# qingpingmo/OCN

Measured on AMD Instinct MI355X. Metric: candidate-edges/sec (CN predictor fwd), ogbl-collab shape, higher is better.
Workload: dtype f32

## Files before the change

### include/ocn_hip.h

```cpp
#ifndef OCN_HIP_H
#define OCN_HIP_H

#include <stdint.h>

#ifdef __cplusplus
extern "C" {
#endif

#define OCN_ABI_VERSION 9
#define OCN_EINVAL (-1)
#define OCN_ECAP   (-2)

#define OCN_ST_CAP  1
#define OCN_ST_SCAN 2
#define OCN_SCAN_POISON (-1)

#define OCN_F_CN1 1u
#define OCN_F_CN2 2u

int ocn_abi_version(void);

int64_t ocn_scan_workspace_bytes(int64_t n);

int ocn_zero_regions(void* const* ptrs, const int64_t* bytes, int32_t n, void* stream);

int ocn_edge_offsets(const int64_t* rowptrA, const int64_t* src, int64_t B,
                     int64_t* off, void* workspace, void* stream);

int ocn_check_edges(const int64_t* src, const int64_t* dst, int64_t B, int64_t n_src, int64_t n_dst,
                    int32_t* bad, void* stream);

int64_t ocn_order_workspace_bytes(int64_t n_nodes);
int ocn_order_by_node(const int64_t* node, int64_t B, int64_t n_nodes, int64_t* order, void* workspace,
                      void* stream);

int ocn_batch_prep(const int64_t* rowptrA, const int64_t* src, int64_t B, int64_t* off , void* scan_workspace,
                   int64_t n_nodes, void* order_workspace , void* const* zero_ptrs, const int64_t* zero_bytes,
                   int32_t n_zero, void* stream);
int ocn_order_by_node_finish(const int64_t* node, int64_t B, int64_t n_nodes, int64_t* order, void* workspace,
                             void* stream);
int ocn_order_by_node_finish_rec(const int64_t* node , const int64_t* dst, const int64_t* rowptrA,
                                 const int64_t* off, int64_t B, int64_t n_nodes, int64_t* order, uint64_t* rec ,
                                 void* workspace, void* stream);

int ocn_chunk_offsets(const int64_t* rowptrA, const int64_t* nds , const int64_t* src,
                      const int64_t* order, int64_t B, int64_t* out, void* workspace, void* stream);

#define OCN_CLASS_RANGES 7
int ocn_class_order(const int32_t* cnt1, const int32_t* cnt2 , const int64_t* order_in ,
                    int64_t B, int64_t* order_out, int64_t* inv_out, int64_t* ranges, int64_t* prefix,
                    void* workspace, void* stream);

int ocn_scan_i32(const int32_t* in, int64_t n, int64_t* out, void* workspace, void* stream);

int ocn_cn_flags(const int64_t* rowptrA, const int32_t* colA,
                 const int64_t* rowptrT1, const int32_t* colT1,
                 const int64_t* rowptrT2, const int32_t* colT2,
                 const uint32_t* bitmapT1 , int64_t bm1_stride_words,
                 const uint32_t* bitmapT2 , int64_t bm_stride_words,
                 const int64_t* src, const int64_t* dst, const int64_t* order, int64_t B,
                 int64_t n_cols, const int64_t* off, uint8_t* flags, int64_t flags_cap,
                 uint64_t* hist , int32_t* cnt1, int32_t* cnt2,
                 int32_t* status, uint64_t* rec , int32_t* gcost , void* stream);
int ocn_cn_flags_rec(const int64_t* rowptrA, const int32_t* colA,
                     const int64_t* rowptrT1, const int32_t* colT1,
                     const int64_t* rowptrT2, const int32_t* colT2,
                     const uint32_t* bitmapT1 , int64_t bm1_stride_words,
                     const uint32_t* bitmapT2 , int64_t bm_stride_words,
                     const int64_t* src, const int64_t* dst, const int64_t* order, int64_t B,
                     int64_t n_cols, const int64_t* off, uint8_t* flags, int64_t flags_cap,
                     uint64_t* hist , int32_t* cnt1, int32_t* cnt2,
                     int32_t* status, uint64_t* rec , int32_t* gcost , void* stream);

int32_t ocn_walk_chunk(void);
int ocn_cn_walk_flags(const int64_t* rowptrA, const int32_t* colA, const int64_t* nds ,
                      const int64_t* src, const int64_t* dst, const int64_t* order, int64_t B,
                      const int64_t* chunk_off, const int64_t* rev_off , const int64_t* off,
                      int64_t max_row_len ,
                      uint8_t* flags, int32_t* wc, int64_t flags_cap,
                      uint64_t* hist , int32_t* cnt1, int32_t* cnt2,
                      int32_t* status, void* stream);

int ocn_neighbor_degree_sum(const int64_t* rowptr, const int32_t* col, int64_t n_rows, int64_t* out,
                            void* stream);
int ocn_walk_rev_offsets(const int64_t* rowptrA, const int64_t* nds, const int64_t* src, const int64_t* dst,
                         const int64_t* order, int64_t B, int64_t* out , void* workspace,
                         void* stream);

int32_t ocn_walk_prep_max_batch(void);
int ocn_walk_prep(const int64_t* rowptrA, const int64_t* nds , const int64_t* src, const int64_t* dst,
                  int64_t B, int32_t min_share, int64_t* order, int64_t* off, int64_t* chunk_off,
                  int64_t* rev_off , int32_t* g_head , int64_t* g_item_off ,
                  int32_t* g_active , int32_t* meta, int32_t* cnt1,
                  int32_t* cnt2, int32_t* status, int32_t* scal, void* stream);
int ocn_cn_walk_group(const int64_t* rowptrA, const int32_t* colA, const int64_t* src, const int64_t* dst,
                      const int64_t* order, int64_t B, const int32_t* g_head, const int64_t* g_item_off,
                      const int32_t* g_active, int32_t* meta, const int64_t* off, uint8_t* flags, int32_t* wc,
                      int64_t flags_cap, uint64_t* hist, int32_t* cnt1, int32_t* cnt2, void* stream);

int ocn_cn_weights_cn5(uint64_t* hist, int64_t N, const float* innerprod, int32_t* scalars,
                       int32_t valued, const float* s2_exact , void* stream);
int ocn_cn_weights_cn7(uint64_t* hist, int64_t N, float sum_fill, const float* diag1 ,
                       const float* diag2 , void* stream);

int ocn_cn5_column_stats(const uint64_t* hist, int64_t N, int32_t* scalars, void* stream);

int64_t ocn_cn_colsum_workspace_bytes(int64_t N, int64_t flags_cap);
int ocn_cn_colsum_exact(const int64_t* rowptrA, const int32_t* colA, const int64_t* src, int64_t B,
                        const int64_t* off, const uint8_t* flagsA, const uint8_t* flagsB ,
                        const int32_t* wc , int64_t flags_cap, const uint64_t* hist ,
                        int64_t N, const float* innerprod, int32_t* scalars, const float* s2_init ,
                        float* s2 , float* s3 , void* workspace, void* stream);

int ocn_cn_gather(const int64_t* rowptrA, const int32_t* colA,
                  const int64_t* src, const int64_t* dst, const int64_t* order, int64_t B,
                  const int64_t* off, const uint8_t* flags, const int32_t* wc,
                  const float* weights , const float* h, int32_t H, int64_t max_row_len,
                  float* xcn1, float* xcn2, float* xij, const int64_t* out_row,
                  const int32_t* cnt1, const int32_t* cnt2, const uint64_t* rec ,
                  const int32_t* perm , const float* rowsum ,
                  void* stream);
int ocn_cn8_pool(const int64_t* rowptrA, const int32_t* colA,
                 const int64_t* rowptrT1 , const int32_t* colT1 ,
                 const int64_t* rowptrT2 , const int32_t* colT2 ,
                 const uint32_t* bitmapT1 , int64_t bm1_stride_words,
// ... 113 lines not shown
int ocn_combine3(const float* coef, const float* x1, const float* x2, const float* x3, int64_t n,
                 float* out, void* stream);

int ocn_fill_rows(float* dst, int64_t ld, int32_t n_cols, const float* vec, const int64_t* row_range,
                  int64_t max_rows, void* stream);

typedef struct OcnLinearGroup {
  const float* X; int64_t ldX;
  int64_t M;
  const void* Wp;
  const float* bias;
  const float* gamma; const float* beta; float eps;
  int32_t relu;
  const float* scale;
  const float* addend; int64_t ldAdd;
  const float* dotw; const float* dotb;
  float* Y; int64_t ldY;
  const int64_t* row_range;
  const int64_t* y_row_map;
  int32_t add_bcast;
} OcnLinearGroup;

int64_t ocn_linear_panel_bytes(int32_t N, int32_t K);
int ocn_linear_split_weight(const float* W, int32_t N, int32_t K, void* Wp, void* stream);
int ocn_linear_bf16x6(const float* X, int64_t M, int32_t K, const void* Wp, int32_t N,
                      const float* bias, const float* gamma, const float* beta, float eps,
                      int32_t relu, const float* dotw, const float* dotb, float* Y, void* stream);
int ocn_linear_grouped(const OcnLinearGroup* groups, int32_t n_groups, int32_t K, int32_t N, void* stream);

typedef struct OcnHeadsArgs {
  const float* x[3];
  int64_t ldx, B;
  int32_t H;
  const void* p_first[3];
  const void* p_mid[2];
  const void* p_out[3];
  const float* vec;
  const int64_t* ranges;
  const int64_t* y_row_map;
  float* y;
  float* dump;
  const float* cpark;
  float* scratch;
  float eps;
  int32_t ln, b_on_union;
} OcnHeadsArgs;
int32_t ocn_heads_nvec(void);
int32_t ocn_heads_nscal(void);
int64_t ocn_heads_scratch_bytes(int32_t H);
int64_t ocn_heads_const_bytes(int32_t H);
int64_t ocn_heads_panel_bytes(int32_t N, int32_t K);
int ocn_heads_split_weight(const float* W, int32_t N, int32_t K, float scale, void* Wp, void* stream);
int ocn_heads_fused(const OcnHeadsArgs* args, void* stream);
int64_t ocn_heads_small_batch(int64_t max_rows);

int64_t ocn_coo_to_csr_workspace_bytes(int64_t nnz, int64_t n_rows, int32_t symmetrize, int32_t dedupe);
int ocn_coo_to_csr(const int64_t* row, const int64_t* col, int64_t nnz, int64_t n_rows, int64_t n_cols,
                   int32_t symmetrize, int32_t dedupe, int64_t* rowptr, int32_t* col_out, void* workspace,
                   int64_t* result, void* stream);

int64_t ocn_wgrad_workspace_bytes(int64_t B, int32_t N, int32_t K);
int ocn_wgrad(const float* dY, int64_t ldY, const float* X, int64_t ldX, int64_t B, int32_t N, int32_t K,
              float* dW, float* db, void* workspace, void* stream);

int64_t ocn_ln_drop_relu_workspace_bytes(int32_t H);
int ocn_ln_drop_relu_forward(const float* x, const float* gamma , const float* beta , float eps, float p,
                             uint64_t seed, int32_t relu, int64_t rows, int32_t H, float* y, float* stats ,
                             void* stream);
int ocn_ln_drop_relu_backward(const float* g, const float* x, const float* y, const float* stats, const float* gamma ,
                              float p, uint64_t seed, int32_t relu, int64_t rows, int32_t H, float* dx,
                              float* dgamma, float* dbeta, void* workspace, void* stream);
int ocn_dropout_keep_mask(uint64_t seed, float p, int64_t n, uint8_t* out, void* stream);

int64_t ocn_mix3_workspace_bytes(void);
int ocn_mix3_backward(const float* coef, const float* g, const float* x1, const float* x2, const float* x3, int64_t n,
                      float* d1, float* d2, float* d3, float* dcoef, void* workspace, void* stream);

#ifdef __cplusplus
}
#endif
#endif
```

### ocn_amd/_lib.py

```python
from __future__ import annotations

import ctypes
import glob
import os
import subprocess
from ctypes import c_float, c_int32, c_int64, c_void_p

_HERE = os.path.dirname(os.path.abspath(__file__))
_ROOT = os.path.dirname(_HERE)
LIB_PATH = os.environ.get("OCN_LIB_PATH", os.path.join(_HERE, "libocn_hip.so"))
CSRC = os.path.join(_HERE, "csrc")
INCLUDE = os.path.join(_ROOT, "include")

_P = c_void_p
ABI_VERSION = 9
SIGNATURES = {
    "ocn_abi_version": (c_int32, []),
    "ocn_scan_workspace_bytes": (c_int64, [c_int64]),
    "ocn_zero_regions": (c_int32, [_P, _P, c_int32, _P]),
    "ocn_check_edges": (c_int32, [_P, _P, c_int64, c_int64, c_int64, _P, _P]),
    "ocn_edge_offsets": (c_int32, [_P, _P, c_int64, _P, _P, _P]),
    "ocn_class_order": (c_int32, [_P, _P, _P, c_int64, _P, _P, _P, _P, _P, _P]),
    "ocn_scan_i32": (c_int32, [_P, c_int64, _P, _P, _P]),
    "ocn_order_workspace_bytes": (c_int64, [c_int64]),
    "ocn_order_by_node": (c_int32, [_P, c_int64, c_int64, _P, _P, _P]),
    "ocn_order_by_node_finish": (c_int32, [_P, c_int64, c_int64, _P, _P, _P]),
    "ocn_order_by_node_finish_rec": (c_int32, [_P, _P, _P, _P, c_int64, c_int64, _P, _P, _P, _P]),
    "ocn_batch_prep": (c_int32, [_P, _P, c_int64, _P, _P, c_int64, _P, _P, _P, c_int32, _P]),
    "ocn_cn_flags": (c_int32, [_P, _P, _P, _P, _P, _P, _P, c_int64, _P, c_int64, _P, _P, _P, c_int64, c_int64, _P, _P, c_int64, _P,
                               _P, _P, _P, _P, _P, _P]),
    "ocn_cn_flags_rec": (c_int32, [_P, _P, _P, _P, _P, _P, _P, c_int64, _P, c_int64, _P, _P, _P, c_int64, c_int64, _P, _P, c_int64, _P,
                                   _P, _P, _P, _P, _P, _P]),
    "ocn_chunk_offsets": (c_int32, [_P, _P, _P, _P, c_int64, _P, _P, _P]),
    "ocn_walk_chunk": (c_int32, []),
    "ocn_cn_walk_flags": (c_int32, [_P, _P, _P, _P, _P, _P, c_int64, _P, _P, _P, c_int64, _P, _P, c_int64, _P, _P, _P,
                                    _P, _P]),
    "ocn_neighbor_degree_sum": (c_int32, [_P, _P, c_int64, _P, _P]),
    "ocn_walk_prep_max_batch": (c_int32, []),
    "ocn_cn_flags_small_graph_cols": (c_int32, []),
    "ocn_walk_prep": (c_int32, [_P, _P, _P, _P, c_int64, c_int32, _P, _P, _P, _P, _P, _P, _P, _P, _P, _P, _P, _P, _P]),
    "ocn_cn_walk_group": (c_int32, [_P, _P, _P, _P, _P, c_int64, _P, _P, _P, _P, _P, _P, _P, c_int64, _P, _P, _P, _P]),
    "ocn_walk_rev_offsets": (c_int32, [_P, _P, _P, _P, _P, c_int64, _P, _P, _P]),
    "ocn_cn_weights_cn5": (c_int32, [_P, c_int64, _P, _P, c_int32, _P, _P]),
    "ocn_cn5_column_stats": (c_int32, [_P, c_int64, _P, _P]),
    "ocn_cn_colsum_workspace_bytes": (c_int64, [c_int64, c_int64]),
    "ocn_cn_colsum_exact": (c_int32, [_P, _P, _P, c_int64, _P, _P, _P, _P, c_int64, _P, c_int64, _P, _P, _P, _P, _P, _P, _P]),
    "ocn_cn_weights_cn7": (c_int32, [_P, c_int64, c_float, _P, _P, _P]),
    "ocn_cn_gather": (c_int32, [_P, _P, _P, _P, _P, c_int64, _P, _P, _P, _P, _P, c_int32, c_int64, _P, _P, _P, _P, _P,
                                _P, _P, _P, _P, _P]),
    "ocn_cn8_pool": (c_int32, [_P, _P, _P, _P, _P, _P, _P, c_int64, _P, c_int64, _P, _P, _P, c_int64, c_int64, _P, c_int32, _P, _P,
                               _P, _P, _P, _P]),
    "ocn_cn_node_sums": (c_int32, [_P, _P, _P, _P, _P, _P, _P, c_int64, _P, c_int64, _P, _P, _P, c_int64, c_int64, _P, _P, _P, _P, _P,
                                   _P, _P]),
    "ocn_row_diff_stage_cols": (c_int32, []),
    "ocn_row_diff_count": (c_int32, [_P, _P, _P, _P, _P, c_int64, c_int32, _P, _P]),
    "ocn_row_diff_fill": (c_int32, [_P, _P, _P, _P, _P, c_int64, c_int32, _P, _P, _P]),
    "ocn_two_hop_window_cols": (c_int64, []),
    "ocn_two_hop_diff_count": (c_int32, [_P, _P, _P, _P, c_int64, _P, c_int64, c_int32, c_int64, _P, _P]),
    "ocn_two_hop_diff_fill": (c_int32, [_P, _P, _P, _P, c_int64, _P, c_int64, c_int32, c_int64, _P, _P, _P]),
    "ocn_segment_topk_max_k": (c_int32, []),
    "ocn_segment_topk": (c_int32, [_P, _P, c_int64, c_int32, _P, _P, _P]),
    "ocn_philox4x32": (c_int32, [_P, ctypes.c_uint32, ctypes.c_uint32, c_int64, _P, _P]),
    "ocn_complement_count": (c_int32, [_P, _P, c_int64, _P, _P]),
    "ocn_sample_stage_cols": (c_int32, []),
    "ocn_sample_complement_rows": (c_int32, [_P, _P, c_int64, _P, c_int64, c_int64, c_int64, ctypes.c_uint64, _P, _P]),
    "ocn_sample_complement_pairs": (c_int32, [_P, _P, c_int64, _P, c_int64, c_int64, ctypes.c_uint64, _P, _P]),
    "ocn_gather_schedule": (c_int32, [_P, c_int64, c_int64, _P, _P]),
    "ocn_coo_to_csr_workspace_bytes": (c_int64, [c_int64, c_int64, c_int32, c_int32]),
    "ocn_coo_to_csr": (c_int32, [_P, _P, c_int64, c_int64, c_int64, c_int32, c_int32, _P, _P, _P, _P, _P]),
    "ocn_wgrad_workspace_bytes": (c_int64, [c_int64, c_int32, c_int32]),
    "ocn_wgrad": (c_int32, [_P, c_int64, _P, c_int64, c_int64, c_int32, c_int32, _P, _P, _P, _P]),
    "ocn_cn_weights_cn6": (c_int32, [_P, _P, c_int64, _P, _P, _P, _P, _P, _P]),
    "ocn_cn_gather3": (c_int32, [_P, _P, _P, _P, _P, c_int64, _P, _P, _P, _P, _P, _P, _P, c_int32, _P, _P, _P, _P, _P]),
    "ocn_cn_gather3_backward": (c_int32, [_P, _P, _P, _P, _P, c_int64, _P, _P, _P, _P, _P, _P, _P, c_int32, _P, _P, _P, _P, _P, _P]),
    "ocn_cn_gather_backward": (c_int32, [_P, _P, _P, _P, _P, c_int64, _P, _P, _P, _P, _P, c_int32, _P, _P, _P, _P, _P]),
    "ocn_cn_gather_backward_det_workspace_bytes": (c_int64, [c_int64, c_int64, c_int64]),
    "ocn_cn_gather_backward_det": (c_int32, [_P, _P, _P, _P, c_int64, _P, _P, _P, c_int64, _P, _P, c_int64, c_int32, _P, _P, _P, _P,
                                             _P, _P]),
    "ocn_cn_gather_backward_det_keys_offset": (c_int64, [c_int64]),
    "ocn_cn_gather_backward_det_lists": (c_int32, [_P, _P, _P, _P, c_int64, _P, _P, c_int64, c_int64, _P, _P]),
    "ocn_ln_drop_relu_workspace_bytes": (c_int64, [c_int32]),
    "ocn_ln_drop_relu_forward": (c_int32, [_P, _P, _P, c_float, c_float, ctypes.c_uint64, c_int32, c_int64, c_int32, _P, _P, _P]),
    "ocn_ln_drop_relu_backward": (c_int32, [_P, _P, _P, _P, _P, c_float, ctypes.c_uint64, c_int32, c_int64, c_int32, _P, _P, _P, _P, _P]),
    "ocn_dropout_keep_mask": (c_int32, [ctypes.c_uint64, c_float, c_int64, _P, _P]),
    "ocn_mix3_workspace_bytes": (c_int64, []),
    "ocn_mix3_backward": (c_int32, [_P, _P, _P, _P, _P, c_int64, _P, _P, _P, _P, _P, _P]),
    "ocn_spmm_csr": (c_int32, [_P, _P, _P, c_int64, _P, c_int32, _P, _P, c_int32, c_int32, c_int32, _P, _P]),
    "ocn_spmm_csr_max_arg": (c_int32, [_P, _P, _P, c_int64, _P, c_int32, _P, _P, _P]),
    "ocn_spmm_max_backward": (c_int32, [_P, _P, _P, c_int64, _P, _P, c_int32, _P, _P]),
    "ocn_deg_rsqrt": (c_int32, [_P, _P, c_int64, c_float, _P, _P]),
    "ocn_spgemm_max_cols": (c_int64, []),
    "ocn_spgemm_pattern_count": (c_int32, [_P, _P, c_int64, _P, _P, c_int64, _P, _P, c_int64, _P]),
    "ocn_spgemm_pattern_fill": (c_int32, [_P, _P, c_int64, _P, _P, c_int64, _P, _P, _P]),
    "ocn_spgemm_bit_rows": (c_int32, [_P, _P, c_int64, _P, _P, c_int64, _P, c_int64, _P, _P, c_int64, _P]),
    "ocn_dense_from_csr": (c_int32, [_P, _P, c_int64, c_int64, _P, _P, _P]),
    "ocn_dense_block_mm_bits": (c_int32, [_P, _P, c_int64, c_int64, c_int32, c_int32, c_int32, c_int32, c_int32, _P, c_int64, _P]),
    "ocn_bitrows_from_csr": (c_int32, [_P, _P, c_int64, _P, c_int64, _P]),
    "ocn_bitrows_count": (c_int32, [_P, c_int64, c_int64, c_int64, _P, _P]),
    "ocn_bitrows_fill": (c_int32, [_P, c_int64, c_int64, c_int64, _P, _P, _P]),
    "ocn_rows_ln_relu": (c_int32, [_P, _P, _P, c_float, c_int32, c_int64, c_int32, _P, _P]),
    "ocn_fill_rows": (c_int32, [_P, c_int64, c_int32, _P, _P, c_int64, _P]),
    "ocn_combine3": (c_int32, [_P, _P, _P, _P, c_int64, _P, _P]),
    "ocn_linear_panel_bytes": (c_int64, [c_int32, c_int32]),
    "ocn_linear_split_weight": (c_int32, [_P, c_int32, c_int32, _P, _P]),
    "ocn_linear_bf16x6": (c_int32, [_P, c_int64, c_int32, _P, c_int32, _P, _P, _P, c_float, c_int32, _P, _P,
                                    _P, _P]),
    "ocn_linear_grouped": (c_int32, [_P, c_int32, c_int32, c_int32, _P]),
    "ocn_heads_nvec": (c_int32, []),
    "ocn_heads_nscal": (c_int32, []),
    "ocn_heads_scratch_bytes": (c_int64, [c_int32]),
    "ocn_heads_const_bytes": (c_int64, [c_int32]),
    "ocn_heads_panel_bytes": (c_int64, [c_int32, c_int32]),
    "ocn_heads_split_weight": (c_int32, [_P, c_int32, c_int32, c_float, _P, _P]),
    "ocn_heads_fused": (c_int32, [_P, _P]),
    "ocn_heads_small_batch": (c_int64, [c_int64]),
}


class OcnHipError(RuntimeError):
    pass


class OcnLinearGroup(ctypes.Structure):
    _fields_ = [("X", c_void_p), ("ldX", c_int64), ("M", c_int64), ("Wp", c_void_p), ("bias", c_void_p),
                ("gamma", c_void_p), ("beta", c_void_p), ("eps", c_float), ("relu", c_int32),
                ("scale", c_void_p), ("addend", c_void_p), ("ldAdd", c_int64), ("dotw", c_void_p),
                ("dotb", c_void_p), ("Y", c_void_p), ("ldY", c_int64), ("row_range", c_void_p),
                ("y_row_map", c_void_p), ("add_bcast", c_int32)]


class OcnHeadsArgs(ctypes.Structure):
    _fields_ = [("x", c_void_p * 3), ("ldx", c_int64), ("B", c_int64), ("H", c_int32),
                ("p_first", c_void_p * 3), ("p_mid", c_void_p * 2), ("p_out", c_void_p * 3),
                ("vec", c_void_p), ("ranges", c_void_p), ("y_row_map", c_void_p), ("y", c_void_p),
                ("dump", c_void_p), ("cpark", c_void_p), ("scratch", c_void_p), ("eps", c_float), ("ln", c_int32), ("b_on_union", c_int32)]


def sources():
    return sorted(glob.glob(os.path.join(CSRC, "*.hip")))


def build_flags():
    return ["-O3", "--offload-arch=gfx950", "-fPIC", "-std=c++17",
            "-ffp-contract=off",
            "-frecord-command-line",
            f"-I{INCLUDE}", f"-I{CSRC}"]


def build(force: bool = False, verbose: bool = False, jobs: int = None) -> str:
    import hashlib
    from concurrent.futures import ThreadPoolExecutor
    out = LIB_PATH
    hdrs = sorted(glob.glob(os.path.join(CSRC, "*.h"))) + [os.path.join(INCLUDE, "ocn_hip.h")]
    deps = sources() + hdrs + [os.path.abspath(__file__)]
    if not force and os.path.exists(out) and \
            os.path.getmtime(out) >= max(os.path.getmtime(d) for d in deps):
        return out
    hipcc = os.environ.get("HIPCC", "/opt/rocm/bin/hipcc")
    flags = build_flags()
    tag = hashlib.sha1(" ".join(flags).encode()).hexdigest()[:10]
    bdir = os.path.join(CSRC, "_build", tag)
    os.makedirs(bdir, exist_ok=True)
    hdr_time = max(os.path.getmtime(h) for h in hdrs)
    todo, objs = [], []
    for src in sources():
        obj = os.path.join(bdir, os.path.basename(src)[:-4] + ".o")
        objs.append(obj)
# ... 52 lines not shown
```

### ocn_amd/csrc/cn_stage.hip

```cpp
#include "common.h"


template <typename P>
__device__ __forceinline__ bool sorted_has(P a, i64 n, int32_t key) {
  i64 lo = 0, hi = n;
  bool found = false;
  while (lo < hi) {
    const i64 mid = (lo + hi) >> 1;
    const int32_t v = a[mid];
    found |= (v == key);
    if (v < key) lo = mid + 1; else hi = mid;
  }
  return found;
}

__device__ __forceinline__ bool sampled_has(const int32_t* samp, const int32_t* __restrict__ row, i64 n,
                                            int32_t key) {
  int lo = 0, hi = OCN_WAVE;
  while (lo < hi) {
    const int mid = (lo + hi) >> 1;
    if (samp[mid] <= key) lo = mid + 1; else hi = mid;
  }
  if (lo == 0) return false;
  const int s = lo - 1;
  const i64 p0 = ((i64)s * n) >> 6, p1 = ((i64)(s + 1) * n) >> 6;
  return sorted_has(row + p0, p1 - p0, key);
}

#define T1_CAP 1024
#define REC_FULL2_BIT 61
#define SCHED_COST(t, c) ((t) > (c) ? (t) : (c))
constexpr int SCHED_SHIFT = 5;
constexpr int POOL_LPE = 64;
#define SCHED_GROUP OCN_WPB

#define LH_MAX_COLS 8192

__device__ __forceinline__ void wave_lds_sync() {
  __builtin_amdgcn_fence(__ATOMIC_ACQ_REL, "wavefront");
  __builtin_amdgcn_wave_barrier();
}
__device__ __forceinline__ i64 wave_uniform(i64 v) {
  const unsigned lo = __builtin_amdgcn_readfirstlane((unsigned)(u64)v), hi = __builtin_amdgcn_readfirstlane((unsigned)((u64)v >> 32));
  return (i64)(((u64)hi << 32) | lo);
}
__device__ __forceinline__ bool lanes_have(int32_t t, int32_t key) {
  int pos = 0;
#pragma unroll
  for (int step = OCN_WAVE / 2; step > 0; step >>= 1)
    if (__shfl(t, pos + step - 1, OCN_WAVE) < key) pos += step;
  return __shfl(t, pos, OCN_WAVE) == key;
}

template <bool HAS_T2, bool LH, bool RECIN>
__global__ __launch_bounds__(OCN_BLOCK) void cn_flags_kernel(
    const i64* __restrict__ rowptrA, const int32_t* __restrict__ colA,
    const i64* __restrict__ rowptrT1, const int32_t* __restrict__ colT1,
    const i64* __restrict__ rowptrT2, const int32_t* __restrict__ colT2,
    const unsigned* __restrict__ bmT1, i64 bm1_stride, const unsigned* __restrict__ bmT2, i64 bm_stride,
    const i64* __restrict__ src, const i64* __restrict__ dst, const i64* __restrict__ order, i64 B,
    i64 n_cols, const i64* __restrict__ off, uint8_t* __restrict__ flags, i64 cap,
    u64* __restrict__ hist, int32_t* __restrict__ cnt1, int32_t* __restrict__ cnt2,
    int32_t* __restrict__ status, u64* rec, int32_t* __restrict__ gcost) {
  constexpr int GPB = OCN_WPB;
  __shared__ int s_cost[2][GPB];
  __shared__ int32_t s_t1[GPB][T1_CAP];
  __shared__ int32_t s_t2[GPB][OCN_WAVE];
  extern __shared__ __attribute__((aligned(16))) u64 s_hist[];
  const int gl = threadIdx.x % OCN_WAVE, g = __builtin_amdgcn_readfirstlane(threadIdx.x / OCN_WAVE);
  if (blockIdx.x == 0 && threadIdx.x == 0) status_raise(status, off[B], cap);
  const bool void_batch = off[B] < 0;
  if (LH) {
    for (i64 c = threadIdx.x; c < n_cols; c += OCN_BLOCK) s_hist[c] = 0ull;
    __syncthreads();
  }
  int par = 0;
  for (i64 e0 = (i64)blockIdx.x * GPB; e0 < B; e0 += (i64)gridDim.x * GPB, par ^= 1) {
    const i64 slot = e0 + g;
    const bool act = slot < B;
    i64 e = 0, i = 0, j = 0, a0 = 0, da = 0, b0 = 0, db = 0, c0 = 0, dc = 0, base = 0;
    const unsigned* bm_row = nullptr;
    const unsigned* bm1_row = nullptr;
    if (act) {
      if (RECIN) {
        const ulonglong2* rp = reinterpret_cast<const ulonglong2*>(rec + 4 * slot);
        const ulonglong2 ra = rp[0], rb = rp[1];
        e = wave_uniform((i64)ra.x);
        i = wave_uniform((i64)(ra.y & 0xffffffffull)); j = wave_uniform((i64)(ra.y >> 32));
        a0 = wave_uniform((i64)(rb.x & ((1ull << REC_LEN_SHIFT) - 1))); da = wave_uniform((i64)(rb.x >> REC_LEN_SHIFT));
        base = wave_uniform((i64)rb.y);
      } else {
        e = order ? order[slot] : slot;
        i = src[e]; j = dst[e];
        a0 = rowptrA[i]; da = rowptrA[i + 1] - a0;
        base = off[e];
      }
      if (bmT1) bm1_row = bmT1 + j * bm1_stride;
      else { b0 = rowptrT1[j]; db = rowptrT1[j + 1] - b0; }
      if (HAS_T2) {
        if (bmT2) bm_row = bmT2 + j * bm_stride;
        if (rowptrT2 && (LH || !bmT2)) { c0 = rowptrT2[j]; dc = rowptrT2[j + 1] - c0; }
      }
      if (void_batch) { da = 0; db = 0; dc = 0; base = 0; }
    }
    const bool t1_reg = db <= OCN_WAVE, t1_lds = db <= T1_CAP;
    int32_t t1 = 0x7fffffff;
    if (t1_reg) { if (gl < db) t1 = colT1[b0 + gl]; }
    else if (t1_lds)
      for (i64 q = gl; q < db; q += OCN_WAVE) s_t1[g][q] = colT1[b0 + q];
    const bool t2_full = HAS_T2 && rowptrT2 && dc == n_cols;
    if (HAS_T2 && !t2_full && !bmT2) {
      if (dc > OCN_WAVE) s_t2[g][gl] = colT2[c0 + (((i64)gl * dc) >> 6)];
      else if (gl < dc) s_t2[g][gl] = colT2[c0 + gl];
    }
    wave_lds_sync();
    const bool fits = base + da <= cap;
    int c1 = 0, c2 = 0;
    for (i64 p0 = 0; p0 < da; p0 += OCN_WAVE) {
      const i64 p = p0 + gl;
      const bool in = p < da;
      const int32_t k = in ? colA[a0 + p] : 0;
      unsigned w2 = 0;
      if (HAS_T2 && bmT2 && !t2_full && in) w2 = bm_row[k >> 5];
      bool f1;
      if (bmT1) f1 = in && ((bm1_row[k >> 5] >> (k & 31)) & 1u);
      else if (t1_reg) f1 = lanes_have(t1, k) && in;
      else f1 = in && (t1_lds ? sorted_has(&s_t1[g][0], db, k) : sorted_has(colT1 + b0, db, k));
      bool f2 = false;
      if (HAS_T2 && in) {
        if (t2_full) f2 = true;
        else if (bmT2) f2 = (w2 >> (k & 31)) & 1u;
        else f2 = dc > OCN_WAVE ? sampled_has(&s_t2[g][0], colT2 + c0, dc, k) : sorted_has(&s_t2[g][0], dc, k);
      }
      if (fits && in) flags[base + p] = (uint8_t)((f1 ? OCN_F_CN1 : 0u) | (f2 ? OCN_F_CN2 : 0u));
      if (f1 | f2) {
        const u64 inc = (u64)f1 | ((u64)f2 << HF_BITS) | (1ull << (2 * HF_BITS));
        if (LH) atomicAdd(s_hist + k, inc); else atomicAdd(hist + 2 * (i64)k, inc);
      }
      c1 += f1;
      c2 += f2;
    }
    wave_lds_sync();
#pragma unroll
    for (int o = OCN_WAVE / 2; o > 0; o >>= 1) {
      c1 += __shfl_xor(c1, o, OCN_WAVE);
      c2 += __shfl_xor(c2, o, OCN_WAVE);
    }
    if (act && gl == 0) {
      cnt1[e] = c1;
      if (cnt2) cnt2[e] = c2;
      if (rec) {
        u64* r = rec + 4 * slot;
        if (!RECIN) {
          r[0] = (u64)e;
          r[1] = (u64)i | ((u64)j << 32);
        }
        if (!RECIN || void_batch) r[2] = (u64)a0 | ((u64)da << REC_LEN_SHIFT);
        r[3] = (u64)base | ((u64)(da > 0 && (i64)c2 == da) << REC_FULL2_BIT) | ((u64)(c1 > 0) << 62) | ((u64)(c2 > 0) << 63);
      }
    }
    if (gcost) {
      if (gl == 0) s_cost[par][g] = act ? c1 + c2 : 0;
      __syncthreads();
      if (threadIdx.x == 0) {
        int t = 0;
#pragma unroll
        for (int q = 0; q < GPB; ++q) t = SCHED_COST(t, s_cost[par][q]);
// ... 425 lines not shown
      const bool need = (wa[t] != 0.f) | (wb[t] != 0.f);
      unsigned long long m = __ballot(need);
      if (LPE < 64) m = (m >> gbase) & ((1ull << (LPE & 63)) - 1ull);
      while (m) {
        int bsel[UNR];
#pragma unroll
        for (int u = 0; u < UNR; ++u) {
          bsel[u] = m ? (__ffsll((long long)m) - 1) : -1;
          m &= m - 1;
        }
        int32_t kk[UNR];
        float wwa[UNR], wwb[UNR];
        float4 x[UNR][NV];
#pragma unroll
        for (int u = 0; u < UNR; ++u) {
          const int sl = gbase + (bsel[u] < 0 ? 0 : bsel[u]);
          kk[u] = __shfl(k[t], sl, OCN_WAVE);
          wwa[u] = __shfl(wa[t], sl, OCN_WAVE);
          wwb[u] = __shfl(wb[t], sl, OCN_WAVE);
          if (bsel[u] >= 0) {
            const float4* row = h4 + (i64)kk[u] * rowq + gl;
#pragma unroll
            for (int v = 0; v < NV; ++v) x[u][v] = row[v * LPE];
          }
        }
#pragma unroll
        for (int u = 0; u < UNR; ++u) {
          if (bsel[u] >= 0) {
            const f32x2 w = {wwa[u], wwb[u]};
#pragma unroll
            for (int v = 0; v < NV; ++v) {
              axpy_pair(acc[v][0], w, x[u][v].x);
              axpy_pair(acc[v][1], w, x[u][v].y);
              axpy_pair(acc[v][2], w, x[u][v].z);
              axpy_pair(acc[v][3], w, x[u][v].w);
            }
          }
        }
      }
    }
  }
#pragma unroll
  for (int v = 0; v < NV; ++v) {
    acc1[v] = make_float4(acc[v][0].x, acc[v][1].x, acc[v][2].x, acc[v][3].x);
    acc2[v] = make_float4(acc[v][0].y, acc[v][1].y, acc[v][2].y, acc[v][3].y);
  }
}

template <int LPE, int NV>
__device__ __forceinline__ void pool_store(i64 e, i64 i, i64 j, int gl, const float4* __restrict__ h4, i64 rowq,
                                           const float4 (&acc1)[NV], const float4 (&acc2)[NV],
                                           float* __restrict__ xcn1, float* __restrict__ xcn2,
                                           float* __restrict__ xij, bool st1 = true, bool st2 = true) {
  const float4* hi = h4 + i * rowq + gl;
  const float4* hj = h4 + j * rowq + gl;
  float4* o1 = reinterpret_cast<float4*>(xcn1) + e * rowq + gl;
  float4* o2 = reinterpret_cast<float4*>(xcn2) + e * rowq + gl;
  float4* o3 = reinterpret_cast<float4*>(xij) + e * rowq + gl;
#pragma unroll
  for (int v = 0; v < NV; ++v) {
    const float4 a = hi[v * LPE], b = hj[v * LPE];
    if (st1) o1[v * LPE] = acc1[v];
    if (st2) o2[v * LPE] = acc2[v];
    o3[v * LPE] = make_float4(__fmul_rn(a.x, b.x), __fmul_rn(a.y, b.y), __fmul_rn(a.z, b.z),
                              __fmul_rn(a.w, b.w));
  }
}

#define LONG_ROW 1024

template <int LPE, int NV>
__global__ __launch_bounds__(OCN_BLOCK) void cn_gather_kernel(
    const i64* __restrict__ rowptrA, const int32_t* __restrict__ colA,
    const i64* __restrict__ src, const i64* __restrict__ dst, const i64* __restrict__ order, i64 B,
    const i64* __restrict__ off, const uint8_t* __restrict__ flags, const int32_t* __restrict__ wc,
    const float4* __restrict__ weights, const float* __restrict__ h, int H,
    float* __restrict__ xcn1, float* __restrict__ xcn2, float* __restrict__ xij,
    const i64* __restrict__ out_row,
    const int32_t* __restrict__ cnt1, const int32_t* __restrict__ cnt2,
    const u64* __restrict__ rec,
    const int32_t* __restrict__ perm,
    const float* __restrict__ rowsum) {
  constexpr int GPW = OCN_WAVE / LPE;
  const int lane = threadIdx.x & 63;
  const int gl = lane % LPE;
  const int gbase = lane - gl;
  i64 bid = blockIdx.x;
  if ((gridDim.x & 7) == 0) {
    bid = (bid & 7) * (gridDim.x >> 3) + (bid >> 3);
    if (perm) bid = perm[bid];
  }
  const i64 slot = (bid * OCN_WPB + (threadIdx.x >> 6)) * GPW + lane / LPE;
  if (slot >= B) return;
  i64 e, i, j, a0, da, base;
  bool has1, has2, full2;
  if (rec) {
    const ulonglong2* rp = reinterpret_cast<const ulonglong2*>(rec + 4 * slot);
    const ulonglong2 ra = rp[0], rb = rp[1];
    e = (i64)ra.x; i = (i64)(ra.y & 0xffffffffull); j = (i64)(ra.y >> 32);
    a0 = (i64)(rb.x & ((1ull << REC_LEN_SHIFT) - 1)); da = (i64)(rb.x >> REC_LEN_SHIFT);
    base = (i64)(rb.y & ((1ull << REC_FULL2_BIT) - 1)); has1 = (rb.y >> 62) & 1ull; has2 = rb.y >> 63;
    full2 = rowsum && ((rb.y >> REC_FULL2_BIT) & 1ull);
  } else {
    e = order ? order[slot] : slot;
    i = src[e]; j = dst[e];
    a0 = rowptrA[i]; da = rowptrA[i + 1] - a0;
    base = off[e];
    has1 = !cnt1 || cnt1[e] > 0; has2 = !cnt2 || cnt2[e] > 0;
    full2 = rowsum && cnt2 && da > 0 && (i64)cnt2[e] == da;
  }
  if (da > LONG_ROW && !full2) return;
  const float4* h4 = reinterpret_cast<const float4*>(h);
  const i64 rowq = H >> 2;
  float4 acc1[NV], acc2[NV];
#pragma unroll
  for (int v = 0; v < NV; ++v) acc1[v] = acc2[v] = make_float4(0.f, 0.f, 0.f, 0.f);
  if (has1 | (has2 & !full2)) pool_range<LPE, NV>(0, da, a0, base, gl, gbase, colA, flags, wc, weights, h4, rowq, acc1, acc2, full2);
  if (full2) {
    const float4* rs = reinterpret_cast<const float4*>(rowsum) + i * rowq + gl;
#pragma unroll
    for (int v = 0; v < NV; ++v) acc2[v] = rs[v * LPE];
  }
  pool_store<LPE, NV>(out_row ? out_row[e] : e, i, j, gl, h4, rowq, acc1, acc2, xcn1, xcn2, xij,
                      !out_row || has1, !out_row || has1 || has2);
}

template <int FPL, int HF>
__device__ __forceinline__ void chain_rows(const float2* __restrict__ w, const float* __restrict__ xs, int nr,
                                           float (&acc1)[FPL], float (&acc2)[FPL]) {
  constexpr int BLK = FPL >= 4 ? 2 : 8 / FPL;
  f32x2 acc[FPL];
#pragma unroll
  for (int q = 0; q < FPL; ++q) acc[q] = f32x2{acc1[q], acc2[q]};
  auto load = [&](int r, float2 (&w8)[BLK], float (&x8)[BLK][FPL]) {
#pragma unroll
    for (int u = 0; u < BLK; ++u) {
      w8[u] = w[r + u];
#pragma unroll
      for (int q = 0; q < FPL; ++q) x8[u][q] = xs[(r + u) * HF + q];
    }
  };
  auto add = [&](const float2 (&w8)[BLK], const float (&x8)[BLK][FPL]) {
#pragma unroll
    for (int u = 0; u < BLK; ++u)
#pragma unroll
      for (int q = 0; q < FPL; ++q) axpy_pair_lds(acc[q], f32x2{w8[u].x, w8[u].y}, x8[u][q]);
  };
  const int nb = nr / BLK;
  if (nb > 0) {
    float2 wa[BLK], wb[BLK];
    float xa[BLK][FPL], xb[BLK][FPL];
    load(0, wa, xa);
    int b = 0;
    for (; b + 2 <= nb; b += 2) {
      load((b + 1) * BLK, wb, xb);
      add(wa, xa);
      if (b + 2 < nb) load((b + 2) * BLK, wa, xa);
      add(wb, xb);
    }
    if (b < nb) add(wa, xa);
  }
  for (int r = nb * BLK; r < nr; ++r) {
    const float2 wr = w[r];
#pragma unroll
// ... 179 lines not shown
    if (f) entry_weights(f, weights[k], (float)cv, wa, wb);
    const bool need = (wa != 0.f) | (wb != 0.f);
    const unsigned long long m = __ballot(need);
    if (lane == 0) s_wcnt[wv] = __popcll(m);
    __syncthreads();
    int before = 0, n = 0;
#pragma unroll
    for (int q = 0; q < WAVES; ++q) {
      const int c = s_wcnt[q];
      if (q < wv) before += c;
      n += c;
    }
    if (need) {
      const int rank = before + __popcll(m & ((1ull << lane) - 1ull));
      s_k[rank] = k;
      s_w[rank] = make_float2(wa, wb);
    }
    __syncthreads();
    const int nsr = (n + SLAB - 1) / SLAB;
    f32x4 xa[RPG][NV], xb[RPG][NV];
    if (wv > 0) {
      long_request<LPE, NV, RPG, FG, SLAB>(xa, s_k, 0, n, fg, gl, h4, rowq);
      long_request<LPE, NV, RPG, FG, SLAB>(xb, s_k, 1, n, fg, gl, h4, rowq);
    }
    for (int t = -1; t < nsr; t += 2) {
      if (wv > 0) {
        long_store<LPE, NV, RPG, FG, SLAB>(xa, s_x + (size_t)((t + 1) & 1) * SLAB * ROWQ, n - (t + 1) * SLAB, fg, gl);
        long_request<LPE, NV, RPG, FG, SLAB>(xa, s_k, t + 3, n, fg, gl, h4, rowq);
      } else if (t >= 0 && lane < AL) {
        const int r0 = t * SLAB;
        chain_rows<FPL, HF>(s_w + r0, reinterpret_cast<const float*>(s_x + (size_t)(t & 1) * SLAB * ROWQ) + lane * FPL,
                            n - r0 < SLAB ? n - r0 : SLAB, acc1, acc2);
      }
      __syncthreads();
      if (t + 1 < nsr) {
        if (wv > 0) {
          long_store<LPE, NV, RPG, FG, SLAB>(xb, s_x + (size_t)((t + 2) & 1) * SLAB * ROWQ, n - (t + 2) * SLAB, fg, gl);
          long_request<LPE, NV, RPG, FG, SLAB>(xb, s_k, t + 4, n, fg, gl, h4, rowq);
        } else if (lane < AL) {
          const int r0 = (t + 1) * SLAB;
          chain_rows<FPL, HF>(s_w + r0, reinterpret_cast<const float*>(s_x + (size_t)((t + 1) & 1) * SLAB * ROWQ) + lane * FPL,
                              n - r0 < SLAB ? n - r0 : SLAB, acc1, acc2);
        }
        __syncthreads();
      }
    }
  }
  if (wv == 0 && lane < AL) {
    const i64 o = (out_row ? out_row[e] : e) * H + lane * FPL;
#pragma unroll
    for (int q = 0; q < FPL; ++q) {
      xcn1[o + q] = acc1[q];
      xcn2[o + q] = acc2[q];
      xij[o + q] = __fmul_rn(h[i * H + lane * FPL + q], h[j * H + lane * FPL + q]);
    }
  }
}

template <int LPE, int NV>
__global__ __launch_bounds__(OCN_BLOCK) void cn_gather3_kernel(
    const i64* __restrict__ rowptrA, const int32_t* __restrict__ colA,
    const i64* __restrict__ src, const i64* __restrict__ dst, const i64* __restrict__ order, i64 B,
    const i64* __restrict__ off, const uint8_t* __restrict__ flagsA, const uint8_t* __restrict__ flagsB,
    const float4* __restrict__ wA, const float4* __restrict__ wB, const float* __restrict__ nip_p,
    const float* __restrict__ h, int H, float* __restrict__ xcn1, float* __restrict__ xcn2,
    float* __restrict__ xcn3, float* __restrict__ xij) {
  constexpr int GPW = OCN_WAVE / LPE;
  constexpr int UNR = 4;
  const int lane = threadIdx.x & 63;
  const int gl = lane % LPE;
  const int gbase = lane - gl;
  const i64 slot = ((i64)blockIdx.x * OCN_WPB + (threadIdx.x >> 6)) * GPW + lane / LPE;
  if (slot >= B) return;
  const i64 e = order ? order[slot] : slot;
  const i64 i = src[e], j = dst[e];
  const i64 a0 = rowptrA[i], da = rowptrA[i + 1] - a0;
  const i64 base = off[e];
  const float nip = nip_p[0];
  const float4* h4 = reinterpret_cast<const float4*>(h);
  const i64 rowq = H >> 2;
  float4 acc1[NV], acc2[NV], acc3[NV];
#pragma unroll
  for (int v = 0; v < NV; ++v) acc1[v] = acc2[v] = acc3[v] = make_float4(0.f, 0.f, 0.f, 0.f);
  for (i64 p0 = 0; p0 < da; p0 += LPE) {
    const i64 p = p0 + gl;
    int32_t k = 0;
    unsigned fa = 0, fb = 0;
    if (p < da) { k = colA[a0 + p]; fa = flagsA[base + p]; fb = flagsB[base + p] & OCN_F_CN1; }
    float w1 = 0.f, w2 = 0.f, w3 = 0.f;
    if (fa | fb) {
      const float4 a = wA[k];
      const float inv3 = wB[k].x;
      const float tt = (fa & OCN_F_CN1) ? a.y : 0.f;
      w1 = (fa & OCN_F_CN1) ? a.x : 0.f;
      w2 = __fmul_rn(__fsub_rn((fa & OCN_F_CN2) ? 1.0f : 0.f, tt), a.z);
      w3 = __fmul_rn(__fsub_rn(__fsub_rn(fb ? 1.0f : 0.f, tt), __fmul_rn(nip, w2)), inv3);
    }
    const bool need = (w1 != 0.f) | (w2 != 0.f) | (w3 != 0.f);
    unsigned long long m = __ballot(need);
    if (LPE < 64) m = (m >> gbase) & ((1ull << (LPE & 63)) - 1ull);
    while (m) {
      int bsel[UNR];
#pragma unroll
      for (int u = 0; u < UNR; ++u) {
        bsel[u] = m ? (__ffsll((long long)m) - 1) : -1;
        m &= m - 1;
      }
// ... 224 lines not shown
      hipLaunchKernelGGL((cn_gather_wave_kernel<LPE, NV>), dim3((unsigned)((B + WW - 1) / WW)),
                         dim3(WW * OCN_WAVE), 0, st, (const i64*)rowptrA, colA, (const i64*)src, (const i64*)dst,
                         (const i64*)order, (i64)B, (const i64*)off, flags, wc, (const float4*)weights, h, (int)H,
                         xcn1, xcn2, xij, (const i64*)out_row, cnt2, rowsum);
      packed = false;
    }
  }
#define PACKED_ARGS (const i64*)rowptrA, colA, (const i64*)src, (const i64*)dst, (const i64*)order, (i64)B, \
                    (const i64*)off, flags, wc, (const float4*)weights, h, (int)H, xcn1, xcn2, xij,           \
                    (const i64*)out_row, cnt1, cnt2, (const u64*)rec
  if (packed)
    hipLaunchKernelGGL((cn_gather_kernel<LPE, NV>), dim3((unsigned)((B + epb - 1) / epb)), dim3(OCN_BLOCK), 0, st,
                       PACKED_ARGS, sched ? perm : (const int32_t*)nullptr, rowsum);
#undef PACKED_ARGS
#define LONG_ARGS (const i64*)rowptrA, colA, (const i64*)src, (const i64*)dst, (i64)B, (const i64*)off, flags, wc, \
                  (const float4*)weights, h, (int)H, xcn1, xcn2, xij, (const i64*)out_row, cnt2, rowsum
  if (max_row_len > LONG_ROW) {
    bool small = false;
    if constexpr (NV == 1) {
      if (B <= 4096) {
        static bool raised_dev[64] = {};
        int devid = 0;
        if (hipGetDevice(&devid) == hipSuccess && devid >= 0 && devid < 64 && !raised_dev[devid]) {
          if (hipFuncSetAttribute((const void*)cn_gather_long_kernel<LPE, NV, LONG_SMALL_THREADS>, hipFuncAttributeMaxDynamicSharedMemorySize,
                                  2 * LONG_SLAB_BYTES(LONG_SMALL_THREADS)) == hipSuccess) raised_dev[devid] = true;
        }
        hipLaunchKernelGGL((cn_gather_long_kernel<LPE, NV, LONG_SMALL_THREADS>), dim3((unsigned)B), dim3(LONG_SMALL_THREADS), 2 * LONG_SLAB_BYTES(LONG_SMALL_THREADS), st, LONG_ARGS);
        small = true;
      }
    }
    if (!small) {
      bool by_wave = false;
      if constexpr (LPE <= 16) {
        hipLaunchKernelGGL((cn_gather_wave_kernel<LPE, NV, true>), dim3((unsigned)B), dim3(OCN_WAVE), 0, st, (const i64*)rowptrA, colA, (const i64*)src, (const i64*)dst,
                           (const i64*)order, (i64)B, (const i64*)off, flags, wc, (const float4*)weights, h, (int)H,
                           xcn1, xcn2, xij, (const i64*)out_row, cnt2, rowsum);
        by_wave = true;
      }
      if (!by_wave) hipLaunchKernelGGL((cn_gather_long_kernel<LPE, NV, 256>), dim3((unsigned)B), dim3(256), 2 * LONG_SLAB_BYTES(256), st, LONG_ARGS);
    }
  }
#undef LONG_ARGS
}

extern "C" {

int32_t ocn_cn_flags_small_graph_cols(void) { return LH_MAX_COLS; }

static int cn_flags_launch(const int64_t* rowptrA, const int32_t* colA, const int64_t* rowptrT1,
                           const int32_t* colT1, const int64_t* rowptrT2, const int32_t* colT2,
                           const uint32_t* bitmapT1, int64_t bm1_stride_words, const uint32_t* bitmapT2, int64_t bm_stride_words,
                           const int64_t* src, const int64_t* dst, const int64_t* order, int64_t B,
                           int64_t n_cols, const int64_t* off, uint8_t* flags, int64_t flags_cap, uint64_t* hist,
                           int32_t* cnt1, int32_t* cnt2, int32_t* status, uint64_t* rec, int32_t* gcost, bool rec_in, void* stream) {
  if (B < 0 || flags_cap < 0 || B > (int64_t)HF_MASK) return OCN_EINVAL;
  if (B == 0) return 0;
  if (!rowptrA || (!rowptrT1 && !bitmapT1) || !src || !dst || !off || !hist || !cnt1 || !status) return OCN_EINVAL;
  if (rec_in && (!rec || !order)) return OCN_EINVAL;
  if ((bitmapT1 && bm1_stride_words * 32 < n_cols) || (bitmapT2 && bm_stride_words * 32 < n_cols)) return OCN_EINVAL;
  constexpr int GPB = OCN_WPB;
  hipStream_t st = (hipStream_t)stream;
  const bool lh = n_cols > 0 && n_cols <= LH_MAX_COLS;
  const size_t lds = lh ? (size_t)n_cols * sizeof(u64) : 0;
  const int grid = lh ? grid_for((B + GPB - 1) / GPB, 256 * 3) : grid_for((B + GPB - 1) / GPB);
  if (lh) {
    static bool raised_dev[64] = {};
    int devid = 0;
    if (hipGetDevice(&devid) != hipSuccess || devid < 0 || devid >= 64) return OCN_EINVAL;
    bool& raised = raised_dev[devid];
    if (!raised) {
      const void* fns[4] = {(const void*)cn_flags_kernel<true, true, false>, (const void*)cn_flags_kernel<false, true, false>,
                            (const void*)cn_flags_kernel<true, true, true>, (const void*)cn_flags_kernel<false, true, true>};
      for (const void* fn : fns) {
        hipError_t e1 = hipFuncSetAttribute(fn, hipFuncAttributeMaxDynamicSharedMemorySize, LH_MAX_COLS * (int)sizeof(u64));
        if (e1 != hipSuccess) return (int)e1;
      }
      raised = true;
    }
  }
#define CN_FLAGS_ARGS(T2P, T2C)                                                                      \
  (const i64*)rowptrA, colA, (const i64*)rowptrT1, colT1, (const i64*)(T2P), (T2C),                   \
      (const unsigned*)bitmapT1, (i64)bm1_stride_words, (const unsigned*)bitmapT2, (i64)bm_stride_words, (const i64*)src, \
      (const i64*)dst, (const i64*)order, (i64)B, (i64)n_cols, (const i64*)off, flags, (i64)flags_cap, \
      (u64*)hist, cnt1, cnt2, status, (u64*)rec, gcost
#define CN_FLAGS_LAUNCH(T2, LHV, RI, T2P, T2C)                                                        \
  hipLaunchKernelGGL((cn_flags_kernel<T2, LHV, RI>), dim3(grid), dim3(OCN_BLOCK), (LHV) ? lds : 0, st, CN_FLAGS_ARGS(T2P, T2C))
#define CN_FLAGS_PICK(T2, T2P, T2C)                                                                   \
  do {                                                                                                \
    if (lh) { if (rec_in) CN_FLAGS_LAUNCH(T2, true, true, T2P, T2C); else CN_FLAGS_LAUNCH(T2, true, false, T2P, T2C); }   \
    else { if (rec_in) CN_FLAGS_LAUNCH(T2, false, true, T2P, T2C); else CN_FLAGS_LAUNCH(T2, false, false, T2P, T2C); }    \
  } while (0)
  if (!rowptrT2 && bitmapT2 && lh) return OCN_EINVAL;
  if (rowptrT2 || bitmapT2) CN_FLAGS_PICK(true, rowptrT2, colT2);
  else CN_FLAGS_PICK(false, nullptr, (const int32_t*)nullptr);
#undef CN_FLAGS_PICK
#undef CN_FLAGS_LAUNCH
  return launch_status();
}

int ocn_cn_flags(const int64_t* rowptrA, const int32_t* colA, const int64_t* rowptrT1,
                 const int32_t* colT1, const int64_t* rowptrT2, const int32_t* colT2,
                 const uint32_t* bitmapT1, int64_t bm1_stride_words, const uint32_t* bitmapT2, int64_t bm_stride_words,
                 const int64_t* src, const int64_t* dst, const int64_t* order, int64_t B,
                 int64_t n_cols, const int64_t* off, uint8_t* flags, int64_t flags_cap, uint64_t* hist,
                 int32_t* cnt1, int32_t* cnt2, int32_t* status, uint64_t* rec, int32_t* gcost, void* stream) {
  return cn_flags_launch(rowptrA, colA, rowptrT1, colT1, rowptrT2, colT2, bitmapT1, bm1_stride_words, bitmapT2, bm_stride_words,
                         src, dst, order, B, n_cols, off, flags, flags_cap, hist, cnt1, cnt2, status, rec, gcost, false, stream);
}

int ocn_cn_flags_rec(const int64_t* rowptrA, const int32_t* colA, const int64_t* rowptrT1,
                     const int32_t* colT1, const int64_t* rowptrT2, const int32_t* colT2,
                     const uint32_t* bitmapT1, int64_t bm1_stride_words, const uint32_t* bitmapT2, int64_t bm_stride_words,
                     const int64_t* src, const int64_t* dst, const int64_t* order, int64_t B,
                     int64_t n_cols, const int64_t* off, uint8_t* flags, int64_t flags_cap, uint64_t* hist,
                     int32_t* cnt1, int32_t* cnt2, int32_t* status, uint64_t* rec, int32_t* gcost, void* stream) {
  return cn_flags_launch(rowptrA, colA, rowptrT1, colT1, rowptrT2, colT2, bitmapT1, bm1_stride_words, bitmapT2, bm_stride_words,
                         src, dst, order, B, n_cols, off, flags, flags_cap, hist, cnt1, cnt2, status, rec, gcost, true, stream);
}

int ocn_cn_walk_flags(const int64_t* rowptrA, const int32_t* colA, const int64_t* nds, const int64_t* src,
                      const int64_t* dst, const int64_t* order, int64_t B, const int64_t* chunk_off,
                      const int64_t* rev_off, const int64_t* off, int64_t max_row_len, uint8_t* flags, int32_t* wc,
                      int64_t flags_cap, uint64_t* hist, int32_t* cnt1, int32_t* cnt2, int32_t* status,
                      void* stream) {
  if (B < 0 || flags_cap < 0 || B > (int64_t)HF_MASK) return OCN_EINVAL;
  if (B == 0) return 0;
  if (!rowptrA || !src || !dst || !chunk_off || !off || !hist || !cnt1 || !cnt2 || !status) return OCN_EINVAL;
  if (flags_cap > 0 && (!flags || !wc)) return OCN_EINVAL;
  if ((nds == nullptr) != (rev_off == nullptr)) return OCN_EINVAL;
  hipStream_t st = (hipStream_t)stream;
  (void)max_row_len;
  const int grid = grid_for(4 * B, 256 * 4);
  if (nds && flags_cap > 0) {
    hipLaunchKernelGGL(walk_zero_kernel, dim3(grid_for((flags_cap + OCN_BLOCK - 1) / OCN_BLOCK, 2048)),
                       dim3(OCN_BLOCK), 0, st, (const i64*)off, (i64)B, (i64)flags_cap, wc);
    hipLaunchKernelGGL(cn_walk_rev_kernel, dim3(grid), dim3(WALK_THREADS), 0, st,
                       (const i64*)rowptrA, colA, (const i64*)src, (const i64*)dst, (const i64*)order, (i64)B,
                       (const i64*)rev_off, (const i64*)off, wc, (i64)flags_cap, status + 2);
  }
  hipLaunchKernelGGL(cn_walk_kernel, dim3(grid), dim3(WALK_THREADS), 0, st,
                     (const i64*)rowptrA, colA, (const i64*)nds, (const i64*)src,
                     (const i64*)dst, (const i64*)order, (i64)B, (const i64*)chunk_off, (const i64*)off, flags, wc,
                     (i64)flags_cap, (u64*)hist, cnt1, cnt2, status);
  return launch_status();
}

int ocn_neighbor_degree_sum(const int64_t* rowptr, const int32_t* col, int64_t n_rows, int64_t* out, void* stream) {
  if (n_rows < 0 || (n_rows > 0 && (!rowptr || !out))) return OCN_EINVAL;
  if (n_rows == 0) return 0;
  hipLaunchKernelGGL(neighbor_degree_sum_kernel, dim3(grid_for((n_rows + OCN_WPB - 1) / OCN_WPB, 1 << 16)),
                     dim3(OCN_BLOCK), 0, (hipStream_t)stream, (const i64*)rowptr, col, (i64)n_rows, (i64*)out);
  return launch_status();
}

int32_t ocn_walk_chunk(void) { return WALK_CHUNK; }

int ocn_cn5_column_stats(const uint64_t* hist, int64_t N, int32_t* scalars, void* stream) {
  if (N < 0 || (N > 0 && (!hist || !scalars))) return OCN_EINVAL;
  if (N == 0) return 0;
  const int grid = grid_for((N + OCN_BLOCK - 1) / OCN_BLOCK, 512);
  hipLaunchKernelGGL(cn5_column_stats, dim3(grid), dim3(OCN_BLOCK), 0, (hipStream_t)stream, (const u64*)hist, (i64)N,
                     scalars);
  return launch_status();
}

int ocn_cn_weights_cn5(uint64_t* hist, int64_t N, const float* innerprod, int32_t* scalars,
                       int32_t valued, const float* s2_exact, void* stream) {
  if (N < 0 || (N > 0 && (!hist || !innerprod || !scalars))) return OCN_EINVAL;
  if (N == 0) return 0;
  const int grid = grid_for((N + OCN_BLOCK - 1) / OCN_BLOCK, 2048);
// ... 33 lines not shown
                                                                    int32_t* __restrict__ perm) {
  __shared__ unsigned short tc[SCHED_BUCKETS * OCN_BLOCK];
  __shared__ i64 s_scan[2 * OCN_WPB];
  const int t = threadIdx.x;
  const i64 lo = (i64)blockIdx.x * per;
  const i64 ipt = (per + OCN_BLOCK - 1) / OCN_BLOCK;
  for (int b = 0; b < SCHED_BUCKETS; ++b) tc[b * OCN_BLOCK + t] = 0;
  auto bucket = [&](i64 q) -> int {
    const int c = max(gcost[lo + q], 0) >> SCHED_SHIFT;
    return SCHED_BUCKETS - 1 - (c < SCHED_BUCKETS - 1 ? c : SCHED_BUCKETS - 1);
  };
  for (i64 k = 0; k < ipt; ++k) {
    const i64 q = (i64)t * ipt + k;
    if (q < per) tc[bucket(q) * OCN_BLOCK + t] += 1;
  }
  __syncthreads();
  i64 mine = 0;
  for (int q = 0; q < SCHED_BUCKETS; ++q) mine += tc[t * SCHED_BUCKETS + q];
  i64 tot;
  i64 run = block_excl_scan(mine, s_scan, &tot);
  for (int q = 0; q < SCHED_BUCKETS; ++q) {
    const int v = tc[t * SCHED_BUCKETS + q];
    tc[t * SCHED_BUCKETS + q] = (unsigned short)run;
    run += v;
  }
  __syncthreads();
  for (i64 k = 0; k < ipt; ++k) {
    const i64 q = (i64)t * ipt + k;
    if (q < per) {
      const int b = bucket(q);
      perm[lo + tc[b * OCN_BLOCK + t]++] = (int32_t)(lo + q);
    }
  }
}

int ocn_gather_schedule(const int32_t* gcost, int64_t n_groups, int64_t segment, int32_t* perm, void* stream) {
  if (n_groups < 0 || (n_groups & 7) || (n_groups >> 3) > 65535 || segment < 0) return OCN_EINVAL;
  if (n_groups == 0) return 0;
  if (!gcost || !perm) return OCN_EINVAL;
  i64 per = n_groups >> 3;
  if (segment > 0 && segment < per && per % segment == 0) per = segment;
  hipLaunchKernelGGL(gather_schedule_kernel, dim3((unsigned)(n_groups / per)), dim3(OCN_BLOCK), 0, (hipStream_t)stream, gcost, per, perm);
  return launch_status();
}

int ocn_cn_gather(const int64_t* rowptrA, const int32_t* colA, const int64_t* src,
                  const int64_t* dst, const int64_t* order, int64_t B, const int64_t* off, const uint8_t* flags,
                  const int32_t* wc, const float* weights, const float* h, int32_t H,
                  int64_t max_row_len, float* xcn1, float* xcn2, float* xij, const int64_t* out_row,
                  const int32_t* cnt1, const int32_t* cnt2, const uint64_t* rec, const int32_t* perm, const float* rowsum,
                  void* stream) {
  if (B < 0 || H <= 0) return OCN_EINVAL;
  if (B == 0) return 0;
  if (!rowptrA || !src || !dst || !off || !weights || !h || !xcn1 || !xcn2 || !xij) return OCN_EINVAL;
  if (rowsum && (wc || !cnt2)) return OCN_EINVAL;
  hipStream_t st = (hipStream_t)stream;
  switch (H) {
    case 16:  LAUNCH_GATHER(4, 1); break;
    case 32:  LAUNCH_GATHER(8, 1); break;
    case 64:  LAUNCH_GATHER(16, 1); break;
    case 128: LAUNCH_GATHER(32, 1); break;
    case 256: LAUNCH_GATHER(POOL_LPE, (64 / POOL_LPE)); break;
    case 512: LAUNCH_GATHER(64, 2); break;
    default:
      hipLaunchKernelGGL(cn_gather_generic, dim3((unsigned)((B + OCN_WPB - 1) / OCN_WPB)),
                         dim3(OCN_BLOCK), 0, st, GATHER_ARGS);
  }
  return launch_status();
}

#define LAUNCH_GATHER3(LPE, NV)                                                                      \
  hipLaunchKernelGGL((cn_gather3_kernel<LPE, NV>),                                                   \
                     dim3((unsigned)((B + (i64)OCN_WPB * (OCN_WAVE / (LPE)) - 1) / ((i64)OCN_WPB * (OCN_WAVE / (LPE))))), \
                     dim3(OCN_BLOCK), 0, (hipStream_t)stream, (const i64*)rowptrA, colA, (const i64*)src,      \
                     (const i64*)dst, (const i64*)order, (i64)B, (const i64*)off, flagsA, flagsB,             \
                     (const float4*)weightsA, (const float4*)weightsB, nip, h, (int)H, xcn1, xcn2, xcn3, xij)

int ocn_cn_gather3(const int64_t* rowptrA, const int32_t* colA, const int64_t* src, const int64_t* dst,
                   const int64_t* order, int64_t B, const int64_t* off, const uint8_t* flagsA,
                   const uint8_t* flagsB, const float* weightsA, const float* weightsB, const float* nip,
                   const float* h, int32_t H, float* xcn1, float* xcn2, float* xcn3, float* xij, void* stream) {
  if (B < 0 || H <= 0) return OCN_EINVAL;
  if (B == 0) return 0;
  if (!rowptrA || !src || !dst || !off || !weightsA || !weightsB || !nip || !h || !xcn1 || !xcn2 || !xcn3 || !xij)
    return OCN_EINVAL;
  switch (H) {
    case 16:  LAUNCH_GATHER3(4, 1); break;
    case 32:  LAUNCH_GATHER3(8, 1); break;
    case 64:  LAUNCH_GATHER3(16, 1); break;
    case 128: LAUNCH_GATHER3(32, 1); break;
    case 256: LAUNCH_GATHER3(64, 1); break;
    case 512: LAUNCH_GATHER3(64, 2); break;
    default: return OCN_EINVAL;
  }
  return launch_status();
}

#define SCATTER_ARGS (const i64*)rowptrA, colA, (const i64*)src, (const i64*)dst, (const i64*)order, (i64)B, \
                     (const i64*)off, flags, wc, (const float4*)weights, h, (int)H, g1, g2, g3, dh
#define LAUNCH_SCATTER(LPE, NV)                                                                     \
  do {                                                                                              \
    const i64 epb = (i64)OCN_WPB * (OCN_WAVE / (LPE));                                              \
    hipLaunchKernelGGL((cn_scatter_kernel<LPE, NV>), dim3((unsigned)((B + epb - 1) / epb)),         \
                       dim3(OCN_BLOCK), 0, (hipStream_t)stream, SCATTER_ARGS);                      \
  } while (0)

int ocn_cn_gather_backward(const int64_t* rowptrA, const int32_t* colA, const int64_t* src,
// ... 51 lines not shown
```

### ocn_amd/csrc/heads.hip

```cpp
#include "common.h"
#include <type_traits>
#include <utility>

typedef __attribute__((ext_vector_type(8))) _Float16 h16x8;
typedef __attribute__((ext_vector_type(16))) float f32x16;
typedef __attribute__((ext_vector_type(4))) unsigned u32x4;
typedef __attribute__((address_space(3))) unsigned char* lds_bytes_t;

#define HD_ROWS 128
#define HD_NVEC 17
#define HD_NSCAL 16
enum { V_B0A = 0, V_B3A, V_G3A, V_E3A, V_B0B, V_B3B, V_G3B, V_E3B, V_B0X, V_GX, V_EX, V_BF, V_GL, V_EL, V_DOTW, V_CA, V_CB };
enum { P_A0 = 0, P_A3, P_MA, P_B0, P_B3, P_MB, P_X0, P_MC, HD_NPANEL };

struct HeadsArgs {
  const float* x[3];
  i64 ldx, B;
  const char* panel[HD_NPANEL];
  const float* vec;
  const i64* ranges;
  const i64* y_row_map;
  float* y;
  float* dump;
  const float* cpark;
  float* scratch;
  float eps;
  int ln, b_on_union;
};

template <typename F, int... I>
__device__ __forceinline__ void hd_unroll_impl(F&& f, std::integer_sequence<int, I...>) {
  (f(std::integral_constant<int, I>{}), ...);
}
template <int N, typename F>
__device__ __forceinline__ void hd_unroll(F&& f) { hd_unroll_impl(f, std::make_integer_sequence<int, N>{}); }


#define HD_WAIT "s_waitcnt lgkmcnt(%[n])\n\t"
#define HD_MF0 "v_mfma_f32_32x32x16_f16 %[c], %[a], %[b], 0\n\t"
#define HD_MFA "v_mfma_f32_32x32x16_f16 %[c], %[a], %[b], %[c]\n\t"
#define HD_RD "ds_read_b128 %[nf], %[ad] offset:%[off]\n\t"
#define HD_SP1 "v_mul_f32 %[t0], %[x0], %[sc]\n\tv_mul_f32 %[t1], %[x1], %[sc]\n\tv_cvt_pk_f16_f32 %[H], %[t0], %[t1]\n\tv_cvt_f32_f16 %[t2], %[H]\n\t"
#define HD_SP2 "v_cvt_f32_f16_sdwa %[t3], %[H] dst_sel:DWORD dst_unused:UNUSED_PAD src0_sel:WORD_1\n\t" \
               "v_sub_f32 %[t0], %[t0], %[t2]\n\tv_sub_f32 %[t1], %[t1], %[t3]\n\tv_cvt_pk_f16_f32 %[L], %[t0], %[t1]\n\t"
#define HD_DMA "s_add_u32 m0, %[ld], %[imm]\n\ts_nop 0\n\tglobal_load_lds_dwordx4 %[vo], %[gb]\n\t"

template <bool CZ, int N, bool PF, int OFF, bool SP>
__device__ __forceinline__ void hd_s1(f32x16& c, const h16x8& a, const h16x8& b, h16x8& nf, unsigned ad, float x0, float x1, float sc,
                                      unsigned& H, float& t0, float& t1, float& t2) {
  static_assert(OFF >= 0 && OFF < 65536 && N >= 0 && N < 16, "immediates");
#define HD_S1(MF, CC, RD, SP1, OUTS, INS) asm volatile(HD_WAIT MF RD SP1 : [c] CC(c) OUTS : [a] "v"(a), [b] "v"(b), [n] "i"(N) INS)
#define HD_O_RD , [nf] "=&v"(nf)
#define HD_I_RD , [ad] "v"(ad), [off] "i"(OFF)
#define HD_O_SP , [H] "=&v"(H), [t0] "=&v"(t0), [t1] "=&v"(t1), [t2] "=&v"(t2)
#define HD_I_SP , [x0] "v"(x0), [x1] "v"(x1), [sc] "v"(sc)
  if constexpr (CZ) {
    if constexpr (PF && SP) HD_S1(HD_MF0, "=a", HD_RD, HD_SP1, HD_O_RD HD_O_SP, HD_I_RD HD_I_SP);
    else if constexpr (PF) HD_S1(HD_MF0, "=a", HD_RD, "", HD_O_RD, HD_I_RD);
    else if constexpr (SP) HD_S1(HD_MF0, "=a", "", HD_SP1, HD_O_SP, HD_I_SP);
    else HD_S1(HD_MF0, "=a", "", "", , );
  } else {
    if constexpr (PF && SP) HD_S1(HD_MFA, "+a", HD_RD, HD_SP1, HD_O_RD HD_O_SP, HD_I_RD HD_I_SP);
    else if constexpr (PF) HD_S1(HD_MFA, "+a", HD_RD, "", HD_O_RD, HD_I_RD);
    else if constexpr (SP) HD_S1(HD_MFA, "+a", "", HD_SP1, HD_O_SP, HD_I_SP);
    else HD_S1(HD_MFA, "+a", "", "", , );
  }
#undef HD_S1
}

template <bool PF, int OFF, bool SP>
__device__ __forceinline__ void hd_s2(f32x16& c, const h16x8& a, const h16x8& b, h16x8& nf, unsigned ad, unsigned H, float& t0, float& t1,
                                      float t2, unsigned& L) {
  static_assert(OFF >= 0 && OFF < 65536, "immediates");
  float t3;
// ... 216 lines not shown
        const int fo = 32 * t + 8 * g + 4 * hh;
        f32x4 y = __builtin_elementwise_fma(in[4 * t + g] * (f32x4)(rstd), hd_lds4(gm + fo), hd_lds4(bt + fo));
        y = __builtin_elementwise_max(y, (f32x4)(0.f));
        m = hd_max4(m, y);
        in[4 * t + g] = y;
      }
    return m;
  }

  static __device__ __forceinline__ void park_share(f32x4* pk_, Acc& acc, float inv, int lane) {
    __attribute__((address_space(1))) f32x4* pk = (__attribute__((address_space(1))) f32x4*)pk_;
#pragma unroll
    for (int t = 0; t < NT; ++t) {
#pragma unroll
      for (int g = 0; g < 4; ++g) pk[(4 * t + g) * 64 + lane] = HD_GRP(acc[t], g) * (f32x4)(inv);
      if (t + 1 < NT) asm volatile("" : "+a"(acc[t + 1]) : : "memory");
    }
  }
};

#define HD_PARK_BYTES(H) ((int64_t)HD_MAX_GRID * 4 * 2 * (H) * 32 * 4)
#define HD_MAX_GRID 256

template <int NT, bool LN>
__global__ __launch_bounds__(OCN_BLOCK, 1) void heads_fused_kernel(const HeadsArgs a) {
  using HD = Heads<NT>;
  using Ring = typename HD::Ring;
  constexpr int H = HD::H, NPW = HD::NPW, CHB = HD::CHB;
  extern __shared__ __attribute__((aligned(16))) unsigned char smem[];
  float* s_vec = reinterpret_cast<float*>(smem);
  const float* s_scal = s_vec + HD_NVEC * H;
  const int lane = threadIdx.x & 63;
  const int w = __builtin_amdgcn_readfirstlane(threadIdx.x >> 6);
  const int r = lane & 31, hh = lane >> 5;
  const unsigned lane16 = (unsigned)lane * 16u;
  const unsigned lds0 = (unsigned)(size_t)(lds_bytes_t)smem;
  for (int q = threadIdx.x; q < HD::VEC_FLOATS; q += OCN_BLOCK) s_vec[q] = a.vec[q];
  const i64 n_tiles = a.dump ? 1 : (a.B + HD_ROWS - 1) / HD_ROWS;
  i64 m3 = a.B, m32 = a.B, m321 = a.B;
  if (a.ranges) { m3 = a.ranges[2 * 1 + 1]; m32 = a.ranges[2 * 0 + 1]; m321 = a.ranges[2 * 3 + 1]; }
  auto tile_runs = [&](i64 tl, int br) -> bool {
    const i64 lo = tl * HD_ROWS, hi = lo + HD_ROWS < a.B ? lo + HD_ROWS : a.B;
    if (br == 0) return lo < m32;
    if (br == 1) return a.b_on_union ? lo < m321 : (lo < m3 || (lo > m32 ? lo : m32) < (hi < m321 ? hi : m321));
    return true;
  };
  auto row_has = [&](i64 slot, int br) -> bool {
    if (slot >= a.B) return false;
    if (br == 0) return slot < m32;
    if (br == 1) return a.b_on_union ? slot < m321 : (slot < m3 || (slot >= m32 && slot < m321));
    return true;
  };
  auto x_row = [&](i64 tl, int br) -> const float* {
    const i64 slot = tl * HD_ROWS + 32 * w + r;
    return a.x[br] + (slot < a.B ? slot : a.B - 1) * a.ldx + 4 * hh;
  };
  auto first_branch = [&](i64 tl) -> int { return tile_runs(tl, 0) ? 0 : (tile_runs(tl, 1) ? 1 : 2); };

  auto uni = [](const char* p) -> const char* {
    const unsigned long long v = (unsigned long long)p;
    const unsigned lo = __builtin_amdgcn_readfirstlane((unsigned)v), hi = __builtin_amdgcn_readfirstlane((unsigned)(v >> 32));
    return (const char*)(((unsigned long long)hi << 32) | lo);
  };
  typename HD::In rA;
  typename HD::Acc rB;
  f32x4* park = reinterpret_cast<f32x4*>(const_cast<char*>(uni(reinterpret_cast<const char*>(
      reinterpret_cast<f32x4*>(a.scratch) + ((size_t)(blockIdx.x * 4 + w) * 2) * (NT * 4) * 64))));
  {
    const float* xr = x_row(blockIdx.x, first_branch(blockIdx.x));
    hd_unroll<4 * NT>([&](auto ic) {
      constexpr int i = decltype(ic)::value;
      hd_xload<(32 * (i / 4) + 8 * (i % 4)) * 4>(rA[i], xr);
    });
    HD::xwait(rA);
  }
  auto x_prepare = [&](bool has) -> float {
    float m = 0.f;
#pragma unroll
    for (int t = 0; t < 4 * NT; ++t) {
      rA[t] = has ? rA[t] : (f32x4)(0.f);
      m = hd_max4(m, __builtin_elementwise_abs(rA[t]));
    }
    HD::pin_in(rA);
    return m;
  };

  auto tile_at = [&](i64 q) -> i64 {
    const i64 G = gridDim.x;
    const i64 t = q * G + ((q & 1) ? G - 1 - (i64)blockIdx.x : (i64)blockIdx.x);
    return t < n_tiles ? t : -1;
  };
#pragma unroll 1
  for (i64 round = 0;; ++round) {
    const i64 tile = tile_at(round);
    if (tile < 0) break;
    const i64 slot = tile * HD_ROWS + 32 * w + r;
    const bool live = slot < a.B;
    const int wgA = tile_runs(tile, 0), wgB = tile_runs(tile, 1);
    const i64 ntile = tile_at(round + 1) >= 0 ? tile_at(round + 1) : tile;
    __syncthreads();

    Ring rg;
#pragma unroll
    for (int k = 0; k < 3; ++k) {
      rg.pa[k] = lds0 + (unsigned)HD::LDS_W + (unsigned)(k * CHB) + lane16;
      rg.ld[k] = lds0 + (unsigned)HD::LDS_W + (unsigned)(k * CHB) + (unsigned)w * 1024u;
    }
    {
// ... 269 lines not shown
#pragma unroll
      for (int ss = 0; ss < 2; ++ss) {
        unsigned xh[4], xl[4];
#pragma unroll
        for (int p = 0; p < 4; ++p) split(y[u][2 * ss + (p >> 1)][2 * (p & 1)], y[u][2 * ss + (p >> 1)][2 * (p & 1) + 1], sc, xh[p], xl[p]);
        const int s = 2 * (w * TW + u) + ss;
        ob[(2 * s) * 64] = hd_frag(xh);
        ob[(2 * s + 1) * 64] = hd_frag(xl);
      }
    __syncthreads();
  }
};


template <int NT, bool LN>
__global__ __launch_bounds__(OCN_BLOCK, 1) void heads_nsplit_kernel(const HeadsArgs a) {
  using HD = Heads<NT>;
  using HN = HeadsN<NT>;
  using panel_t = typename HN::panel_t;
  constexpr int H = HD::H, TW = HN::TW, PD = HN::PD, ROWS = HN::ROWS;
  extern __shared__ __attribute__((aligned(16))) unsigned char smem[];
  float* s_vec = reinterpret_cast<float*>(smem);
  const float* s_scal = s_vec + HD_NVEC * H;
  const int lane = threadIdx.x & 63;
  const int w = __builtin_amdgcn_readfirstlane(threadIdx.x >> 6);
  const int r = lane & 31, hh = lane >> 5;
  h16x8* ob = reinterpret_cast<h16x8*>(smem + HD::LDS_W) + lane;
  float* red = reinterpret_cast<float*>(smem + HD::LDS_W + (size_t)HN::OB_VECS * 16);
  for (int q = threadIdx.x; q < HD::VEC_FLOATS; q += OCN_BLOCK) s_vec[q] = a.vec[q];
  i64 m3 = a.B, m32 = a.B, m321 = a.B;
  if (a.ranges) { m3 = a.ranges[2 * 1 + 1]; m32 = a.ranges[2 * 0 + 1]; m321 = a.ranges[2 * 3 + 1]; }
  const i64 tile = blockIdx.x;
  const i64 lo = tile * ROWS, hi = lo + ROWS < a.B ? lo + ROWS : a.B;
  const i64 slot = lo + r;
  const bool live = slot < a.B;
  const bool wgA = lo < m32;
  const bool wgB = a.b_on_union ? lo < m321 : (lo < m3 || (lo > m32 ? lo : m32) < (hi < m321 ? hi : m321));
  auto row_has = [&](int br) -> bool {
    if (!live) return false;
    if (br == 0) return slot < m32;
    if (br == 1) return a.b_on_union ? slot < m321 : (slot < m3 || (slot >= m32 && slot < m321));
    return true;
  };
  auto panel = [&](int P) -> const char* { return a.panel[P]; };
  const unsigned vo = (unsigned)(w * TW * 2048 + lane * 16);
  typename HN::Acc acc;
  typename HN::Frag fr;
  typename HN::Own xin[3];
  const int br0 = wgA ? 0 : (wgB ? 1 : 2);
  {
#pragma unroll
    for (int br = 0; br < 3; ++br) {
      if (!(br == 0 ? wgA : (br == 1 ? wgB : true))) continue;
      const float* xr = a.x[br] + (live ? slot : a.B - 1) * a.ldx + 4 * hh + 32 * (w * TW);
#pragma unroll
      for (int u = 0; u < TW; ++u)
#pragma unroll
        for (int g = 0; g < 4; ++g) xin[br][u][g] = *reinterpret_cast<const f32x4*>(xr + 32 * u + 8 * g);
    }
    const char* p0 = panel(br0 == 2 ? P_X0 : 3 * br0);
    hd_unroll<PD>([&](auto kc) { HN::template fetch<decltype(kc)::value>(fr, vo, p0); });
  }
  auto zero_unless = [&](typename HN::Own& y, bool has) {
#pragma unroll
    for (int u = 0; u < TW; ++u)
#pragma unroll
      for (int g = 0; g < 4; ++g) y[u][g] = has ? y[u][g] : (f32x4)(0.f);
  };
  __syncthreads();
  f32x4 sab[TW][4];
#pragma unroll
  for (int u = 0; u < TW; ++u)
#pragma unroll
    for (int g = 0; g < 4; ++g) sab[u][g] = (f32x4)(-0.f);
  typedef const __attribute__((address_space(1))) f32x4* gf4_t;
  const gf4_t ck = (gf4_t)reinterpret_cast<const f32x4*>(a.cpark);
  typename HN::Own y;
  float inv;
  HN::drain(fr);
#pragma unroll
  for (int br = 0; br < 2; ++br) {
    if (!(br == 0 ? wgA : wgB)) {
#pragma unroll
      for (int u = 0; u < TW; ++u)
#pragma unroll
        for (int g = 0; g < 4; ++g) sab[u][g] += ck[(size_t)(br * 4 * NT + 4 * (w * TW + u) + g) * 64 + lane];
      continue;
    }
    const float* vb = s_vec + (br == 0 ? V_B0A : V_B0B) * H;
    const char *p0 = panel(3 * br), *p1 = panel(3 * br + 1), *p2 = panel(3 * br + 2);
    const int nbr = (br == 0 && wgB) ? 1 : 2;
    const char* pn = panel(nbr == 2 ? P_X0 : 3 * nbr);
    zero_unless(xin[br], row_has(br));
    HN::template operand<true>(ob, xin[br], s_scal[1 + 3 * br], inv, red, w, lane);
    HN::template layer<false>(acc, ob, fr, vo, p0, p1);
    HN::template bias<true>(y, acc, inv, vb, w, hh);
    HN::template operand<false>(ob, y, s_scal[2 + 3 * br], inv, red, w, lane);
    HN::template layer<false>(acc, ob, fr, vo, p1, p2);
    HN::template bias<!LN>(y, acc, inv, vb + H, w, hh);
    if constexpr (LN) HN::ln_relu(y, vb + 2 * H, vb + 3 * H, a.eps, red, w, hh, lane);
    HN::template operand<false>(ob, y, s_scal[3 + 3 * br], inv, red, w, lane);
    HN::template layer<false>(acc, ob, fr, vo, p2, pn);
#pragma unroll
    for (int u = 0; u < TW; ++u)
#pragma unroll
      for (int g = 0; g < 4; ++g) sab[u][g] += HD_GRP(acc[u], g) * (f32x4)(inv);
    HN::drain(fr);
// ... 90 lines not shown
    raised_dev[devid] = true;
  }
  hipLaunchKernelGGL((heads_fused_kernel<NT, LN>), dim3((unsigned)(tiles < HD_MAX_GRID ? tiles : HD_MAX_GRID)), dim3(OCN_BLOCK),
                     Heads<NT>::LDS_BYTES, st, a);
  return launch_status();
}

template <int NT, bool LN>
static int heads_nsplit_launch(const HeadsArgs& a, hipStream_t st) {
  static bool raised_dev[64] = {};
  int devid = 0;
  if (hipGetDevice(&devid) != hipSuccess || devid < 0 || devid >= 64) return OCN_EINVAL;
  if (!raised_dev[devid]) {
    const hipError_t e = hipFuncSetAttribute((const void*)heads_nsplit_kernel<NT, LN>, hipFuncAttributeMaxDynamicSharedMemorySize,
                                             (int)HeadsN<NT>::LDS_BYTES);
    if (e != hipSuccess) return (int)e;
    raised_dev[devid] = true;
  }
  const i64 tiles = (a.B + HeadsN<NT>::ROWS - 1) / HeadsN<NT>::ROWS;
  hipLaunchKernelGGL((heads_nsplit_kernel<NT, LN>), dim3((unsigned)tiles), dim3(OCN_BLOCK), HeadsN<NT>::LDS_BYTES, st, a);
  return launch_status();
}

static int64_t g_heads_small_batch = 16384;

extern "C" {

int64_t ocn_heads_small_batch(int64_t max_rows) {
  const int64_t prev = g_heads_small_batch;
  if (max_rows >= 0) g_heads_small_batch = max_rows;
  return prev;
}

int64_t ocn_heads_panel_bytes(int32_t N, int32_t K) {
  if (N <= 0 || K <= 0 || (N & 31) || (K & 31)) return 0;
  return (int64_t)N * K * 4;
}

int ocn_heads_split_weight(const float* W, int32_t N, int32_t K, float scale, void* Wp, void* stream) {
  if (!W || !Wp || N <= 0 || K <= 0 || (N & 31) || (K & 31) || !(scale > 0.f)) return OCN_EINVAL;
  const i64 frags = (i64)(K / 16) * (N >> 5) * 64;
  hipLaunchKernelGGL(split_weight_f16_kernel, dim3(grid_for((frags + OCN_BLOCK - 1) / OCN_BLOCK, 1024)),
                     dim3(OCN_BLOCK), 0, (hipStream_t)stream, W, (int)N, (int)K, scale, (h16x8*)Wp);
  return launch_status();
}

int32_t ocn_heads_nvec(void) { return HD_NVEC; }
int32_t ocn_heads_nscal(void) { return HD_NSCAL; }

int64_t ocn_heads_const_bytes(int32_t H) { return (int64_t)2 * H * 32 * 4; }

int64_t ocn_heads_scratch_bytes(int32_t H) { return HD_PARK_BYTES(H) + 4096; }

int ocn_heads_fused(const OcnHeadsArgs* h, void* stream) {
  if (!h || h->B < 0 || h->H <= 0) return OCN_EINVAL;
  if (h->B == 0) return 0;
  for (int i = 0; i < 3; ++i)
    if (!h->x[i] || !h->p_first[i] || !h->p_out[i]) return OCN_EINVAL;
  if (!h->p_mid[0] || !h->p_mid[1] || !h->vec || !h->scratch || (!h->y && !h->dump)) return OCN_EINVAL;
  if (h->dump ? h->B != 1 : !h->cpark) return OCN_EINVAL;
  const int64_t ldx = h->ldx ? h->ldx : h->H;
  if (ldx < h->H || (ldx & 3)) return OCN_EINVAL;
  HeadsArgs a;
  for (int i = 0; i < 3; ++i) a.x[i] = h->x[i];
  a.panel[P_A0] = (const char*)h->p_first[0]; a.panel[P_A3] = (const char*)h->p_mid[0]; a.panel[P_MA] = (const char*)h->p_out[0];
  a.panel[P_B0] = (const char*)h->p_first[1]; a.panel[P_B3] = (const char*)h->p_mid[1]; a.panel[P_MB] = (const char*)h->p_out[1];
  a.panel[P_X0] = (const char*)h->p_first[2]; a.panel[P_MC] = (const char*)h->p_out[2];
  a.ldx = ldx; a.B = h->B; a.vec = h->vec; a.ranges = (const i64*)h->ranges; a.y_row_map = (const i64*)h->y_row_map;
  a.y = h->y; a.dump = h->dump; a.cpark = h->cpark; a.scratch = h->scratch; a.eps = h->eps; a.ln = h->ln; a.b_on_union = h->b_on_union;
  const i64 tiles = h->dump ? 1 : (h->B + HD_ROWS - 1) / HD_ROWS;
  hipStream_t st = (hipStream_t)stream;
  if (!h->dump && h->B <= g_heads_small_batch * (256 / h->H)) switch (h->H) {
      case 128: return h->ln ? heads_nsplit_launch<4, true>(a, st) : heads_nsplit_launch<4, false>(a, st);
      case 256: return h->ln ? heads_nsplit_launch<8, true>(a, st) : heads_nsplit_launch<8, false>(a, st);
      default: return OCN_EINVAL;
    }
  switch (h->H) {
    case 128: return h->ln ? heads_launch<4, true>(a, tiles, st) : heads_launch<4, false>(a, tiles, st);
    case 256: return h->ln ? heads_launch<8, true>(a, tiles, st) : heads_launch<8, false>(a, tiles, st);
    default: return OCN_EINVAL;
  }
}

}
```

### ocn_amd/model.py

```python
from __future__ import annotations

from typing import Final, Iterable, Optional

import torch
import torch.nn as nn
from torch import Tensor

import os

from . import ops
from .sparse import SparseTensor
from .utils import fuse


class DropEdge(nn.Module):
    def __init__(self, dp: float = 0.0) -> None:
        super().__init__()
        self.dp = dp

    def forward(self, edge_index: Tensor):
        if self.dp == 0:
            return edge_index
        mask = torch.rand_like(edge_index[0], dtype=torch.float) > self.dp
        return edge_index[:, mask]
# ... 506 lines not shown
        self.register_parameter("beta", nn.Parameter(beta * torch.ones((1))))
        self.dropadj = DropAdj(edrop)
        H, p = hidden_channels, dropout
        norm = (lambda: nn.LayerNorm(H)) if ln else (lambda: nn.Identity())
        drop = lambda: nn.Dropout(p, inplace=True)
        relu = lambda: nn.ReLU(inplace=True)

        def pooled_head(tail_identity=False):
            return nn.Sequential(nn.Linear(in_channels, H), drop(), relu(), nn.Linear(H, H), norm(),
                                 drop(), relu(), nn.Identity() if tail_identity else nn.Linear(H, H))

        self.xlin = nn.Sequential(nn.Linear(H, H), drop(), relu(), nn.Linear(H, H), norm(), drop(),
                                  relu()) if use_xlin else (lambda x: 0)
        self.xcnlin = pooled_head(tail_identity=tailact)
        self.xcn1lin = pooled_head()
        self.xcn2lin = pooled_head()
        self.xcn4lin = pooled_head()
        self.xijlin = nn.Sequential(nn.Linear(in_channels, H), norm(), drop(), relu(),
                                    nn.Identity() if tailact else nn.Linear(H, H))
        two = twolayerlin
        self.lin = nn.Sequential(nn.Linear(H, H), norm(), drop(), relu(),
                                 nn.Linear(H, H) if two else nn.Identity(),
                                 norm() if two else nn.Identity(),
                                 drop() if two else nn.Identity(),
                                 relu() if two else nn.Identity(),
                                 nn.Linear(H, out_channels))
        self.cndeg = cndeg
        self.register_parameter("alpha", nn.Parameter(torch.ones((3))))
        self.register_buffer("innerprod", torch.tensor([0.0]))
        self.n = 0
        self._shard_group, self._sharded = None, False
        self._ws = {}

    def set_edge_sharding(self, group=None, enabled: bool = True) -> None:
        self._shard_group, self._sharded = group, enabled

    def _exchange(self, st, x=None):
        if self._sharded:
            from .dist import allreduce_hist_finish, allreduce_hist_start
            handle = allreduce_hist_start(st.hist, self._shard_group, valued=st.walk, slice_edges=st.B)
            st.sharded, st.shard_group = True, self._shard_group
            if x is not None:
                self._class_order(st, x)
            allreduce_hist_finish(handle)
            ops._mark("allreduce_hist")
        return st

    def begin(self, x, adj, cn1, cn2, tar_ei, slot: int = 0, args=None):
        if self.training or torch.is_grad_enabled():
            raise RuntimeError("begin / finish is the no-grad scoring path: call .eval() under torch.no_grad()")
        n_sets = max(2, int(ops.overlap_depth), int(ops.overlap_depth_small))
        if len(getattr(self, "_ws_slots", ())) != n_sets:
            self._ws_slots = [dict() for _ in range(n_sets)]
        st = fuse(cn1, cn2, tar_ei, self._ws_slots[slot % n_sets], adj=adj)
        handle = None
        if self._sharded:
            from .dist import allreduce_hist_start
            st.sharded, st.shard_group = True, self._shard_group
            if ops.shard_reduce_in_finish if ops.shard_reduce_in_finish is not None else ops._overlap_active:
                handle = "late"
            else:
                handle = allreduce_hist_start(st.hist, self._shard_group, valued=True, slice_edges=st.B)
        w = None
        if handle is None and not self._sharded:
            if args is not None or not self._weights_need_args:
                w = self._weights(st, args)
            if ops.phase_a_extras:
                self._class_order(st, x)
                st.prepare_schedule(x.shape[1])
                if ops.phase_a_pool and w is not None:
                    st.pooled = self._pool(st, w, x)
        return st, handle, w

    def finish(self, x, token, args=None):
        st, handle, w_early = token
        ops._mark("begin")
        if isinstance(handle, str):
            from .dist import allreduce_hist_start
            handle = allreduce_hist_start(st.hist, self._shard_group, valued=True, slice_edges=st.B)
        if not getattr(st, "_cls_decided", False):
            self._class_order(st, x)
        if handle is not None:
            from .dist import allreduce_hist_finish
            allreduce_hist_finish(handle)
            ops._mark("allreduce_hist")
        pooled = getattr(st, "pooled", None)
        if pooled is None:
            w = w_early if w_early is not None else self._weights(st, args)
            pooled = self._pool(st, w, x)
        xcn1, xcn2, xij = pooled
        return self._heads(x, xcn1, xcn2, xij, getattr(st, "cls", None))

    def check_errors(self) -> None:
        words = [t for d in ([self._ws] + list(getattr(self, "_ws_slots", ()))) for k, t in d.items() if k[0] == "status"]
        if not words:
            return
        bits = 0
        for v in torch.stack([t[3] for t in words]).tolist():
            bits |= int(v)
        if bits:
            for t in words:
                t[3:].zero_()
            raise RuntimeError(ops.status_message(bits))

    def _class_order(self, st, x) -> None:
        st.cls = None
        st._cls_decided = True
        if (ops.skip_zero_rows and not self.training and not torch.is_grad_enabled() and st.B >= ops.skip_zero_min_batch
                and st.cnt2 is not None and (self._fused_plan(x.shape[1]) is not None or self._heads_plan(x.shape[1]) is not None)
                and self._skip_worthwhile()):
            st.cls = ops.class_order(st.cnt1, st.cnt2, st.order, st.ws)
            self._skip_probe(st.cls[2], st.B)

    def _scratch(self, x):
        return None if (torch.is_grad_enabled() and (x.requires_grad or self.training)) else self._ws

    def _pool(self, st, w, x):
        x = x.contiguous()
        if torch.is_grad_enabled() and x.requires_grad:
            return _PoolFn.apply(x, st, w)
        if not getattr(st, "_cls_decided", False):
            self._class_order(st, x)
        rs = self._rowsum(st, x)
        if st.cls is not None:
            return st.gather(w, x, out_row=st.cls[1], rowsum=rs)
        return st.gather(w, x, rowsum=rs)

    def _rowsum(self, st, x):
        return None

    def _skip_worthwhile(self) -> bool:
        pr = getattr(self, "_skip_state", None)
        if pr is None:
            return True
        if torch.cuda.is_current_stream_capturing():
            return pr["off"] == 0
        if pr["pending"] is not None and pr["pending"].query():
            r = pr["host"]
            B = max(int(pr["B"]), 1)
            cn1, any_, none = int(r[ops.R_CN1][1]), int(r[ops.R_ANY][1]), B - int(r[ops.R_ANY][1])
            pr["share"] = ((B - cn1) + 2 * none) / (3.0 * B)
            pr["pending"] = None
            if pr["share"] < ops.skip_zero_min_share:
                pr["off"] = ops.skip_zero_backoff
# ... 178 lines not shown
                    lns = [sa[1][1], sb[1][1], sx[0][1], sl[0][1]]
                    if all(l is None for l in lns) or (all(l is not None for l in lns) and len({l.eps for l in lns}) == 1):
                        plan = (sa, sb, sx, sl[0], tail)
            self._fplan, self._fplan_key = plan, key
        return self._fplan

    def _fused_pack(self, H: int, dev):
        sa, sb, sx, sl, tail = self._fused_plan(H)
        plist = getattr(self, "_fp_params", None)
        if plist is None:
            plist = self._fp_params = [p for seq in (self.xcn1lin, self.xcn2lin, self.xijlin, self.lin) for p in seq.parameters()]
        self._mix_coef()
        key = (tuple(p._version for p in plist), tuple(p.data_ptr() for p in plist), self._coef_key, str(dev))
        if getattr(self, "_fpack_key", None) == key:
            return self._fpack
        with torch.no_grad():
            c = self._mix_coef().double()
            W0l, b0l = sl[0].weight.double(), sl[0].bias.double()
            Ma = c[0] * (W0l @ sa[2][0].weight.double())
            Mb = c[1] * (W0l @ sb[2][0].weight.double())
            bsum = c[0] * sa[2][0].bias.double() + c[1] * sb[2][0].bias.double()
            if len(sx) == 2:
                Mc = c[2] * (W0l @ sx[1][0].weight.double())
                bsum = bsum + c[2] * sx[1][0].bias.double()
            else:
                Mc = c[2] * W0l
            bf = W0l @ bsum + b0l
            ln = sa[1][1] is not None
            zeros, ones = torch.zeros(H, device=dev), torch.ones(H, device=dev)

            def gb(l):
                return (l.weight.float(), l.bias.float()) if l is not None else (ones, zeros)
            vecs = [sa[0][0].bias, sa[1][0].bias, *gb(sa[1][1]), sb[0][0].bias, sb[1][0].bias, *gb(sb[1][1]),
                    sx[0][0].bias, *gb(sx[0][1]), bf.float(), *gb(sl[1]), tail.weight.reshape(-1), zeros, zeros]
            assert len(vecs) == int(ops._lib.lib().ocn_heads_nvec())
            pans = [ops.heads_panel(m.float().contiguous()) for m in
                    (sa[0][0].weight, sa[1][0].weight, Ma, sb[0][0].weight, sb[1][0].weight, Mb, sx[0][0].weight, Mc)]
            nscal = int(ops._lib.lib().ocn_heads_nscal())
            scal = torch.zeros(nscal, device=dev)
            scal[0] = tail.bias.detach().float().reshape(())
            scal[1:9] = torch.tensor([p[1] for p in pans], device=dev)
            vec = torch.cat([v.detach().float().reshape(-1) for v in vecs] + [scal]).contiguous()
            pack = dict(first=[pans[0][0], pans[3][0], pans[6][0]], mid=[pans[1][0], pans[4][0]],
                        out=[pans[2][0], pans[5][0], pans[7][0]],
                        vec=vec, ln=ln, eps=(sa[1][1].eps if ln else 1e-5), flops_per_row=2.0 * H * H * 8)
            z = torch.zeros(1, H, device=dev)
            cpark = torch.empty(int(ops._lib.lib().ocn_heads_const_bytes(H)) // 4, device=dev)
            scratch = ops.buf(self._ws, "heads_scratch", int(ops._lib.lib().ocn_heads_scratch_bytes(H)) // 4, torch.float32, dev)
            ops.heads_fused(z, z, z, pack, None, None, self._xcn2_on_union, scratch, dump=cpark)
            pack["cpark"] = cpark
        self._fpack, self._fpack_key = pack, key
        return pack

    def _heads_fused(self, xcn1, xcn2, xij, cls):
        B, H = xij.shape
        pack = self._fused_pack(H, xij.device)
        scratch = ops.buf(self._ws, "heads_scratch", int(ops._lib.lib().ocn_heads_scratch_bytes(H)) // 4, torch.float32, xij.device)
        ranges, rowmap = (None, None) if cls is None else (cls[2], cls[0])
        return ops.heads_fused(xcn1, xcn2, xij, pack, ranges, rowmap, self._xcn2_on_union, scratch)

    def _heads(self, x, xcn1, xcn2, xij, cls=None):
        if (not self.training and not torch.is_grad_enabled() and xij.is_cuda and xij.dim() == 2 and xij.shape[0] > 0
                and xij.is_contiguous() and xcn1.is_contiguous() and xcn2.is_contiguous()
                and xcn1.shape == xij.shape and xij.shape[1] >= ops.fused_heads_min_width
                and self._fused_plan(xij.shape[1]) is not None):
            return self._heads_fused(xcn1, xcn2, xij, cls)
        if cls is not None:
            return self._heads_skipping(xcn1, xcn2, xij, cls)
        if self.training or torch.is_grad_enabled() or not xij.is_cuda or xij.shape[-1] % 4:
            alpha = torch.sigmoid(self.alpha).cumprod(-1)
            run = _seq_train if (xij.is_cuda and ops.train_linear) else (lambda seq, t: seq(t))
            xij = run(self.xijlin, xij)
            xcn1 = run(self.xcn1lin, xcn1)
            xcn2 = run(self.xcn2lin, xcn2)
            return run(self.lin, _mix(alpha, self.beta, xcn1, xcn2, xij))
        z = self._heads_grouped(xcn1, xcn2, xij)
        if z is not None:
            return _seq_eval(self.lin, z)
        xij = _seq_eval(self.xijlin, xij)
        xcn1 = _seq_eval(self.xcn1lin, xcn1)
        xcn2 = _seq_eval(self.xcn2lin, xcn2)
        z = ops.combine3(self._mix_coef(), xcn1, xcn2, xij)
        return _seq_eval(self.lin, z)


class CNLinkPredictorOringin(_CNPredictorBase):

    def multidomainforward(self, x, adj, cn1, cn2, tar_ei, filled1: bool = False,
                           cndropprobs: Iterable[float] = []):
        st = self._exchange(fuse(cn1, cn2, tar_ei, self._scratch(x), adj=adj), x)
        w = self._weights(st, None)
        xcn1, xcn2, xij = self._pool(st, w, x)
        return self._heads(x, xcn1, xcn2, xij, getattr(st, "cls", None))

    def _weights(self, st, args):
        return st.weights_cn5(self.innerprod1(st))

    def forward(self, x, adj, cn1, cn2, tar_ei, filled1: bool = False):
        return self.multidomainforward(x, adj, cn1, cn2, tar_ei, filled1, [])


class CNLinkPredictorbaselearn(_CNPredictorBase):
    _xcn2_on_union = False
    _weights_need_args = True
    polyfirst: int = 0
    polysecond: int = 0

    def multidomainforward(self, x, adj, cn1, cn2, tar_ei, args, filled1: bool = False,
                           cndropprobs: Iterable[float] = []):
        st = self._exchange(fuse(cn1, cn2, tar_ei, self._scratch(x), adj=adj), x)
        w = self._weights(st, args)
        xcn1, xcn2, xij = self._pool(st, w, x)
        return self._heads(x, xcn1, xcn2, xij, getattr(st, "cls", None))

    def _weights(self, st, args):
        dev = st.hist.device
        return st.weights_cn7(float(args.sum), chebyshev_diag(st.N, int(self.polyfirst), dev),
                              chebyshev_diag(st.N, int(self.polysecond), dev))

    def _rowsum(self, st, x):
        adj, t2 = st.adj, getattr(st, "t2", None)
        if not ops.share_full_rows or st.walk or t2 is None or not x.is_cuda or x.dim() != 2 or int(self.polysecond) != 0:
            return None
        n = adj.size(0)
        if t2.nnz() * 2 < n * n or adj.size(1) != x.shape[0] or n != x.shape[0]:
            return None
        import weakref
        hit = getattr(self, "_rowsum_cache", None)
        if (hit is None or hit[0]() is not x or hit[1] != x._version or hit[2]() is not adj
                or hit[3] != (x.data_ptr(), tuple(x.shape))):
            if torch.cuda.is_current_stream_capturing() and hit is not None:
                raise RuntimeError("embeddings changed since the last eager call: run one eager batch before capturing")
            hit = self._rowsum_cache = (weakref.ref(x), x._version, weakref.ref(adj), (x.data_ptr(), tuple(x.shape)),
                                        ops.spmm_csr(adj._rowptr, adj._col, x))
        return hit[4]

    def forward(self, x, adj, cn1, cn2, tar_ei, filled1: bool = False):
        return self.multidomainforward(x, adj, cn1, cn2, tar_ei, filled1, [])


class CNLinkPredictorbaselearnablation(_CNPredictorBase):
    _xcn2_on_union = False

    def _fused_state(self, x, cn1, cn2, tar_ei, ws):
        if (not ops.cn8_fused_eval or self.training or torch.is_grad_enabled() or not torch.is_tensor(x) or x.dim() != 2
                or x.dtype != torch.float32 or x.shape[1] not in ops.LN_WIDTHS):
            return None
        from .utils import fuse8
        st = fuse8(cn1, cn2, tar_ei, ws)
        if st is not None:
            st.cls, st._cls_decided = None, True
        return st

    def multidomainforward(self, x, adj, cn1, cn2, tar_ei, args, filled1: bool = False,
                           cndropprobs: Iterable[float] = []):
        getattr(args, "sum", None)
        st = self._fused_state(x, cn1, cn2, tar_ei, self._scratch(x))
        if st is not None:
            xcn1, xcn2, xij = st.pool(x.contiguous())
            return self._heads(x, xcn1, xcn2, xij, None)
        st = fuse(cn1, cn2, tar_ei, self._scratch(x), adj=adj)
        xcn1, xcn2, xij = self._pool(st, self._weights(st, args), x)
        return self._heads(x, xcn1, xcn2, xij, getattr(st, "cls", None))

    def _weights(self, st, args):
        return ops.unit_weights(st.N, st.src.device)
# ... 76 lines not shown
```

### ocn_amd/ops.py

```python
from __future__ import annotations

import ctypes
import os
from typing import Optional, Tuple

import torch
from torch import Tensor

from . import _lib
from ._lib import check, ptr, stream_ptr

FLAGS_NOSYNC_LIMIT = 1 << 30
validate_indices = True
stage_timer = None
LN_WIDTHS = (16, 32, 64, 128, 256, 512)
a1_bitmap_max_bytes = int(os.environ.get("OCN_A1_BITMAP_MAX_BYTES", 64 << 20))
a2_bitmap_max_bytes = 16 << 30
skip_zero_rows = True
skip_zero_min_share = 0.15
skip_zero_backoff = 32
skip_zero_min_batch = 4096
walk_two_sided = True
walk_share_min = 2
sort_edges_min_batch = 4096
# ... 124 lines not shown
    check(_lib.lib().ocn_scan_i32(ptr(cnt), n, ptr(out), ptr(ws), stream_ptr()), "ocn_scan_i32")
    return out


@_on_device
def check_edges(src: Tensor, dst: Tensor, n_src: int, n_dst: int) -> None:
    if not validate_indices or src.numel() == 0:
        return
    if (int(n_src), int(n_dst)) in getattr(_checked, "scopes", ()):
        return
    _req(src, torch.int64, "src", 1); _req(dst, torch.int64, "dst", 1)
    bad = torch.zeros(1, dtype=torch.int32, device=src.device)
    check(_lib.lib().ocn_check_edges(ptr(src), ptr(dst), src.numel(), int(n_src), int(n_dst), ptr(bad), stream_ptr()),
          "ocn_check_edges")
    if int(bad.item()):
        raise IndexError("candidate edge endpoint out of range for the adjacency")


import threading
_checked = threading.local()


class prevalidated:

    def __init__(self, src: Tensor, dst: Tensor, n_src: int, n_dst: int):
        check_edges(src.contiguous(), dst.contiguous(), n_src, n_dst)
        self._key = (int(n_src), int(n_dst))

    def __enter__(self):
        if not hasattr(_checked, "scopes"):
            _checked.scopes = []
        _checked.scopes.append(self._key)
        return self

    def __exit__(self, *exc):
        _checked.scopes.remove(self._key)
        return False


HIST_FIELD_BITS = 21
MAX_BATCH = (1 << HIST_FIELD_BITS) - 1


def hist_counts(hist: Tensor) -> Tensor:
    m = (1 << HIST_FIELD_BITS) - 1
    p = hist[:, 0]
    return torch.stack([p & m, (p >> HIST_FIELD_BITS) & m, (p >> (2 * HIST_FIELD_BITS)) & m, hist[:, 1]], dim=1)


@_on_device
def cn_flags(rowptrA: Tensor, colA: Tensor, t1: Optional[Tuple[Tensor, Tensor]],
             t2: Optional[Tuple[Tensor, Tensor]], src: Tensor, dst: Tensor, n_cols: int, max_deg_a: int,
             walk: bool = False, t2_bitmap: Optional[Tensor] = None, wsd=None, nds: Optional[Tensor] = None,
             t1_bitmap: Optional[Tensor] = None, rec: Optional[Tensor] = None, sched: Optional[Tensor] = None):
    dev = src.device
    B = src.numel()
    _req(rowptrA, torch.int64, "rowptrA", 1); _req(colA, torch.int32, "colA", 1)
    if not walk:
        _req(t1[0], torch.int64, "rowptrT1", 1); _req(t1[1], torch.int32, "colT1", 1)
        if t2 is not None:
            if t2[0] is not None or t2_bitmap is None or n_cols <= small_graph_cols():
                _req(t2[0], torch.int64, "rowptrT2", 1)
            if t2[1] is not None or t2_bitmap is None:
                _req(t2[1], torch.int32, "colT2", 1)
    _req(src, torch.int64, "src", 1); _req(dst, torch.int64, "dst", 1)
    if dst.numel() != B:
        raise ValueError("src/dst length mismatch")
    if B > MAX_BATCH:
        raise ValueError(f"candidate batch of {B} edges exceeds the histogram field width ({MAX_BATCH})")
    _mark("begin")
    if walk and 0 < B <= int(_lib.lib().ocn_walk_prep_max_batch()) and walk_share_min > 0:
        return _cn_flags_walk_small(rowptrA, colA, src, dst, n_cols, max_deg_a, wsd, nds)
    want_order = B >= sort_edges_min_batch
    n_src = rowptrA.numel() - 1
    order = buf(wsd, "order", B, torch.int64, dev) if want_order else None
    ows = (buf(wsd, "order_ws", int(_lib.lib().ocn_order_workspace_bytes(n_src)) // 8 + 1, torch.int64, dev, zero_init=True)
           if want_order else None)
    off = buf(wsd, "off", B + 1, torch.int64, dev)
    sws = buf(wsd, "scan_ws", int(_lib.lib().ocn_scan_workspace_bytes(B)) // 8 + 1, torch.int64, dev, zero_init=True)
    hist = buf(wsd, "hist", (n_cols, 2), torch.int64, dev)
    cnt1 = buf(wsd, "cnt1", B, torch.int32, dev)
    cnt2 = buf(wsd, "cnt2", B, torch.int32, dev) if (walk or t2 is not None) else None
    status = buf(wsd, "status", 4, torch.int32, dev, zero_init=True)
    scal = buf(wsd, "scal", 4, torch.int32, dev)
    zs = [t for t in [hist, status[:3], scal] + ([cnt1, cnt2] if walk else []) if t is not None and t.numel()]
    if sched is not None:
        if rec is None or walk or _req(sched, torch.int32, "sched", 1).numel() < 2 * ((B + 3) // 4):
            raise ValueError("sched: int32[2 * ceil(B / 4)] beside the slot records of the pattern route")
    zp = (ctypes.c_void_p * len(zs))(*[t.data_ptr() for t in zs])
    zb = (ctypes.c_int64 * len(zs))(*[t.numel() * t.element_size() for t in zs])
    check(_lib.lib().ocn_batch_prep(ptr(rowptrA), ptr(src), B, ptr(off), ptr(sws), n_src, ptr(ows), zp, zb, len(zs),
                                    stream_ptr()), "ocn_batch_prep")
    rec_in = want_order and rec is not None and not walk
    if rec_in:
        _req(dst, torch.int64, "dst", 1)
        if _req(rec, torch.int64, "rec").numel() < 4 * B:
            raise ValueError("rec: int64 [B, 4]")
        check(_lib.lib().ocn_order_by_node_finish_rec(ptr(src), ptr(dst), ptr(rowptrA), ptr(off), B, n_src, ptr(order), ptr(rec),
                                                      ptr(ows), stream_ptr()), "ocn_order_by_node_finish_rec")
    elif want_order:
        check(_lib.lib().ocn_order_by_node_finish(ptr(src), B, n_src, ptr(order), ptr(ows), stream_ptr()),
              "ocn_order_by_node_finish")
    bound = B * max(int(max_deg_a), 0)
    cap = bound if bound <= FLAGS_NOSYNC_LIMIT else _total(off[-1])
    flags = buf(wsd, "flags", max(cap, 1), torch.uint8, dev)
    wc = buf(wsd, "wc", max(cap, 1), torch.int32, dev) if walk else None
    chunk_off = rev_off = None
    if walk:
        if nds is not None and walk_two_sided:
            _req(nds, torch.int64, "nds", 1)
            if nds.numel() != rowptrA.numel() - 1:
                raise ValueError("nds does not match the adjacency")
        else:
            nds = None
        chunk_off = buf(wsd, "chunk_off", B + 1, torch.int64, dev)
        cws = buf(wsd, "scan_ws", int(_lib.lib().ocn_scan_workspace_bytes(B)) // 8 + 1, torch.int64, dev, zero_init=True)
        check(_lib.lib().ocn_chunk_offsets(ptr(rowptrA), ptr(nds), ptr(src), ptr(order), B, ptr(chunk_off), ptr(cws),
                                           stream_ptr()), "ocn_chunk_offsets")
        if nds is not None:
            rev_off = buf(wsd, "rev_off", B + 1, torch.int64, dev)
            check(_lib.lib().ocn_walk_rev_offsets(ptr(rowptrA), ptr(nds), ptr(src), ptr(dst), ptr(order), B,
                                                  ptr(rev_off), ptr(cws), stream_ptr()), "ocn_walk_rev_offsets")
    _mark("cn_prep")
    if walk:
        check(_lib.lib().ocn_cn_walk_flags(ptr(rowptrA), ptr(colA), ptr(nds), ptr(src), ptr(dst), ptr(order), B,
                                           ptr(chunk_off), ptr(rev_off), ptr(off), int(max_deg_a), ptr(flags),
                                           ptr(wc), cap, ptr(hist), ptr(cnt1), ptr(cnt2), ptr(status),
                                           stream_ptr()), "ocn_cn_walk_flags")
    else:
        if t2_bitmap is not None:
            _req(t2_bitmap, torch.int32, "t2_bitmap", 2)
            if t2 is None or (t2[0] is not None and t2_bitmap.shape[0] != t2[0].numel() - 1) or t2_bitmap.shape[1] * 32 < n_cols:
                raise ValueError("t2_bitmap does not match the T2 adjacency")
        if t1_bitmap is not None:
            _req(t1_bitmap, torch.int32, "t1_bitmap", 2)
            if t1_bitmap.shape[0] != t1[0].numel() - 1 or t1_bitmap.shape[1] * 32 < n_cols:
                raise ValueError("t1_bitmap does not match the T1 adjacency")
        check((_lib.lib().ocn_cn_flags_rec if rec_in else _lib.lib().ocn_cn_flags)(ptr(rowptrA), ptr(colA), ptr(t1[0]), ptr(t1[1]),
                                      ptr(t2[0] if t2 else None), ptr(t2[1] if t2 else None),
                                      ptr(t1_bitmap), t1_bitmap.shape[1] if t1_bitmap is not None else 0,
                                      ptr(t2_bitmap), t2_bitmap.shape[1] if t2_bitmap is not None else 0,
                                      ptr(src), ptr(dst), ptr(order), B, n_cols, ptr(off), ptr(flags), cap, ptr(hist),
                                      ptr(cnt1), ptr(cnt2), ptr(status), ptr(rec), ptr(sched), stream_ptr()), "ocn_cn_flags")
    _mark("cn_flags")
    return order, off, flags, wc, hist, cnt1, cnt2, status, scal


def _cn_flags_walk_small(rowptrA, colA, src, dst, n_cols, max_deg_a, wsd, nds):
    dev, B = src.device, src.numel()
    l = _lib.lib()
    if nds is not None and walk_two_sided:
        _req(nds, torch.int64, "nds", 1)
        if nds.numel() != rowptrA.numel() - 1:
            raise ValueError("nds does not match the adjacency")
    else:
        nds = None
    order = buf(wsd, "order", B, torch.int64, dev)
    off = buf(wsd, "off", B + 1, torch.int64, dev)
    chunk_off = buf(wsd, "chunk_off", B + 1, torch.int64, dev)
    rev_off = buf(wsd, "rev_off", B + 1, torch.int64, dev) if nds is not None else None
    g_head = buf(wsd, "g_head", B + 1, torch.int32, dev)
    g_item_off = buf(wsd, "g_item_off", B + 1, torch.int64, dev)
    g_active = buf(wsd, "g_active", B, torch.int32, dev)
    meta = buf(wsd, "walk_meta", 4, torch.int32, dev)
    hist = buf(wsd, "hist", (n_cols, 2), torch.int64, dev)
    cnt1 = buf(wsd, "cnt1", B, torch.int32, dev)
    cnt2 = buf(wsd, "cnt2", B, torch.int32, dev)
    status = buf(wsd, "status", 4, torch.int32, dev, zero_init=True)
    scal = buf(wsd, "scal", 4, torch.int32, dev)
    check(l.ocn_walk_prep(ptr(rowptrA), ptr(nds), ptr(src), ptr(dst), B, int(walk_share_min), ptr(order), ptr(off),
                          ptr(chunk_off), ptr(rev_off), ptr(g_head), ptr(g_item_off), ptr(g_active), ptr(meta), ptr(cnt1),
                          ptr(cnt2), ptr(status), ptr(scal), stream_ptr()), "ocn_walk_prep")
    zero_regions([hist])
    bound = B * max(int(max_deg_a), 0)
    cap = bound if bound <= FLAGS_NOSYNC_LIMIT else _total(off[-1])
    flags = buf(wsd, "flags", max(cap, 1), torch.uint8, dev)
    wc = buf(wsd, "wc", max(cap, 1), torch.int32, dev)
    _mark("cn_prep")
    check(l.ocn_cn_walk_flags(ptr(rowptrA), ptr(colA), ptr(nds), ptr(src), ptr(dst), ptr(order), B, ptr(chunk_off),
                              ptr(rev_off), ptr(off), int(max_deg_a), ptr(flags), ptr(wc), cap, ptr(hist), ptr(cnt1),
                              ptr(cnt2), ptr(status), stream_ptr()), "ocn_cn_walk_flags")
    check(l.ocn_cn_walk_group(ptr(rowptrA), ptr(colA), ptr(src), ptr(dst), ptr(order), B, ptr(g_head), ptr(g_item_off),
                              ptr(g_active), ptr(meta), ptr(off), ptr(flags), ptr(wc), cap, ptr(hist), ptr(cnt1), ptr(cnt2),
                              stream_ptr()), "ocn_cn_walk_group")
    _mark("cn_flags")
    return order, off, flags, wc, hist, cnt1, cnt2, status, scal


@_on_device
def neighbor_degree_sum(rowptr: Tensor, col: Tensor) -> Tensor:
    _req(rowptr, torch.int64, "rowptr", 1); _req(col, torch.int32, "col", 1)
    n = rowptr.numel() - 1
    out = torch.empty(n, dtype=torch.int64, device=rowptr.device)
    check(_lib.lib().ocn_neighbor_degree_sum(ptr(rowptr), ptr(col), n, ptr(out), stream_ptr()),
          "ocn_neighbor_degree_sum")
    return out
# ... 22 lines not shown

@_on_device
def cn_colsum_exact(rowptrA, colA, src, off, flagsA, flagsB, wc, hist: Tensor, innerprod: Tensor, scal: Tensor, wsd=None,
                    s2_init: Optional[Tensor] = None):
    _req(hist, torch.int64, "hist", 2)
    N, dev = hist.shape[0], hist.device
    cap = flagsA.numel()
    if cap >= (1 << 32) - 1:
        raise NotImplementedError("order-exact column sums address flag positions with 32 bits")
    ip = _req(innerprod.detach().reshape(1).to(torch.float32), torch.float32, "innerprod", 1)
    if s2_init is not None and _req(s2_init, torch.float32, "s2_init", 1).numel() != N:
        raise ValueError("s2_init must have one entry per column")
    s2 = buf(wsd, "s2_exact", N, torch.float32, dev)
    s3 = buf(wsd, "s3_exact", N, torch.float32, dev) if flagsB is not None else None
    ws = buf(wsd, "colsum_ws", int(_lib.lib().ocn_cn_colsum_workspace_bytes(N, cap)) // 8 + 1, torch.int64, dev)
    check(_lib.lib().ocn_cn_colsum_exact(ptr(rowptrA), ptr(colA), ptr(src), src.numel(), ptr(off), ptr(flagsA), ptr(flagsB),
                                         ptr(wc), cap, ptr(hist), N, ptr(ip), ptr(scal), ptr(s2_init), ptr(s2), ptr(s3),
                                         ptr(ws), stream_ptr()), "ocn_cn_colsum_exact")
    _mark("cn_colsum")
    return s2, s3


@_on_device
def cn_weights_cn5(hist: Tensor, innerprod: Tensor, valued: bool = False, wsd=None, s2_exact: Optional[Tensor] = None,
                   scal: Optional[Tensor] = None) -> Tensor:
    _req(hist, torch.int64, "hist", 2)
    ip = _req(innerprod.detach().reshape(1).to(torch.float32), torch.float32, "innerprod", 1)
    if scal is None:
        scal = buf(wsd, "scal", 4, torch.int32, hist.device, zero=True)
    if _ip_nonzero(innerprod) and s2_exact is None:
        check(_lib.lib().ocn_cn5_column_stats(ptr(hist), hist.shape[0], ptr(scal), stream_ptr()), "ocn_cn5_column_stats")
    check(_lib.lib().ocn_cn_weights_cn5(ptr(hist), hist.shape[0], ptr(ip), ptr(scal), int(valued), ptr(s2_exact),
                                        stream_ptr()), "ocn_cn_weights_cn5")
    _mark("cn_weights")
    return hist.view(torch.float32)


@_on_device
def cn_weights_cn7(hist: Tensor, sum_fill: float, diag1: Optional[Tensor] = None, diag2: Optional[Tensor] = None) -> Tensor:
    _req(hist, torch.int64, "hist", 2)
    for d, nm in ((diag1, "diag1"), (diag2, "diag2")):
        if d is not None and _req(d, torch.float32, nm, 1).numel() != hist.shape[0]:
            raise ValueError(f"{nm}: one entry per column")
    check(_lib.lib().ocn_cn_weights_cn7(ptr(hist), hist.shape[0], float(sum_fill), ptr(diag1), ptr(diag2), stream_ptr()),
          "ocn_cn_weights_cn7")
    _mark("cn_weights")
    return hist.view(torch.float32)


@_on_device
def cn_gather(rowptrA, colA, src, dst, off, flags, wc: Optional[Tensor], weights: Tensor, h: Tensor,
              order: Optional[Tensor] = None, max_row_len: int = 0, wsd=None, out_row: Optional[Tensor] = None,
              cnt1: Optional[Tensor] = None, cnt2: Optional[Tensor] = None, rec: Optional[Tensor] = None,
              sched: Optional[Tensor] = None, rowsum: Optional[Tensor] = None, sched_ready: bool = False):
    _req(weights, torch.float32, "weights", 2)
    _req(h, torch.float32, "h", 2)
    if weights.shape[0] != h.shape[0] or weights.shape[1] != 4:
        raise ValueError("weights must be [N,4] with N = h.shape[0]")
    B, H = src.numel(), h.shape[1]
    out = buf(wsd, "pooled", (3, B, H), torch.float32, h.device)
    if rowsum is not None and (wc is not None or cnt2 is None or _req(rowsum, torch.float32, "rowsum", 2).shape != h.shape):
        raise ValueError("rowsum: [N, H] row sums of h, pattern route with per-row counts only")
    perm = None
    if sched is not None and rec is not None and H == 256 and B % 32 == 0 and B // 32 <= 65535:
        n_groups = B // 4
        perm = sched[n_groups:]
        if not sched_ready:
            check(_lib.lib().ocn_gather_schedule(ptr(sched), n_groups, int(sched_segment), ptr(perm), stream_ptr()), "ocn_gather_schedule")
    _mark("cn_pre")
    check(_lib.lib().ocn_cn_gather(ptr(rowptrA), ptr(colA), ptr(src), ptr(dst), ptr(order), B, ptr(off), ptr(flags),
                                   ptr(wc), ptr(weights), ptr(h), H, int(max_row_len), ptr(out[0]), ptr(out[1]),
                                   ptr(out[2]), ptr(out_row), ptr(cnt1), ptr(cnt2), ptr(rec), ptr(perm), ptr(rowsum),
                                   stream_ptr()), "ocn_cn_gather")
    _mark("cn_gather")
    return out[0], out[1], out[2]


_unit_w: dict = {}


def unit_weights(n: int, device) -> Tensor:
    key = (int(n), str(device))
    w = _unit_w.get(key)
    if w is None:
        if len(_unit_w) > 8:
            _unit_w.clear()
        w = _unit_w[key] = torch.tensor([1.0, 0.0, 1.0, 0.0], device=device).repeat(int(n), 1).contiguous()
    return w


@_on_device
def order_by_node(node: Tensor, n_nodes: int, wsd=None) -> Tensor:
    _req(node, torch.int64, "node", 1)
    B = node.numel()
    order = buf(wsd, "order", B, torch.int64, node.device)
    ows = buf(wsd, "order_ws", int(_lib.lib().ocn_order_workspace_bytes(n_nodes)) // 8 + 1, torch.int64, node.device, zero_init=True)
    check(_lib.lib().ocn_order_by_node(ptr(node), B, int(n_nodes), ptr(order), ptr(ows), stream_ptr()), "ocn_order_by_node")
    return order


cn8_fused_eval = os.environ.get("OCN_CN8_FUSED", "0") == "1"


@_on_device
def cn8_pool(rowptrA: Tensor, colA: Tensor, t1: Optional[Tuple[Optional[Tensor], Optional[Tensor]]],
             t2: Optional[Tuple[Optional[Tensor], Optional[Tensor]]], src: Tensor, dst: Tensor, h: Tensor,
             t1_bitmap: Optional[Tensor] = None, t2_bitmap: Optional[Tensor] = None, order: Optional[Tensor] = None, wsd=None,
             n_cols: Optional[int] = None):
    _req(rowptrA, torch.int64, "rowptrA", 1); _req(colA, torch.int32, "colA", 1)
    _req(src, torch.int64, "src", 1); _req(dst, torch.int64, "dst", 1)
    _req(h, torch.float32, "h", 2)
    B, (N, H) = src.numel(), h.shape
    if dst.numel() != B:
        raise ValueError("src/dst length mismatch")
    if H not in LN_WIDTHS:
        raise NotImplementedError(f"cn8 pooling supports hidden widths {LN_WIDTHS}, got {H}")
    if n_cols is not None and int(n_cols) != N:
        raise ValueError(f"h has {N} rows, the adjacency {int(n_cols)} columns")
    csr, n_rows = [], []
    for t, bm, nm in ((t1, t1_bitmap, "T1"), (t2, t2_bitmap, "T2")):
        rp, col = (None, None) if t is None else t
        if rp is None or col is None:
            if bm is None:
                raise ValueError(f"{nm}: needs its CSR arrays or its bit rows")
            rp = col = None
        else:
            _req(rp, torch.int64, "rowptr" + nm, 1); _req(col, torch.int32, "col" + nm, 1)
        if bm is not None:
# ... 639 lines not shown
    _req_strided(dst, "dst")
    _req(vec, torch.float32, "vec")
    _req(row_range, torch.int64, "row_range", 1)
    if vec.numel() != dst.shape[1]:
        raise ValueError("fill_rows: width mismatch")
    check(_lib.lib().ocn_fill_rows(ptr(dst), dst.stride(0), dst.shape[1], ptr(vec), ptr(row_range), dst.shape[0],
                                   stream_ptr()), "ocn_fill_rows")
    _mark("mlp_glue")


LINEAR_WIDTHS = (32, 64, 128, 256)
fast_linear = True
_panels: dict = {}


@_on_device
def linear_panel(weight: Tensor) -> Tensor:
    import weakref
    key = id(weight)
    hit = _panels.get(key)
    if (hit is not None and hit[0]() is weight and hit[1] == weight.data_ptr() and hit[2] == weight._version
            and hit[3] == tuple(weight.shape)):
        return hit[4]
    w = _req(weight.detach(), torch.float32, "weight", 2)
    N, K = w.shape
    panel = torch.empty(int(_lib.lib().ocn_linear_panel_bytes(N, K)), dtype=torch.uint8, device=w.device)
    check(_lib.lib().ocn_linear_split_weight(ptr(w), N, K, ptr(panel), stream_ptr()), "ocn_linear_split_weight")
    if len(_panels) > 512:
        for k in [k for k, v in _panels.items() if v[0]() is None]:
            del _panels[k]
    _panels[key] = (weakref.ref(weight), weight.data_ptr(), weight._version, (N, K), panel)
    return panel


@_on_device
def heads_panel(weight: Tensor):
    import math
    w = _req(weight.detach(), torch.float32, "weight", 2)
    N, K = w.shape
    m = float(w.abs().max().item()) if w.numel() else 0.0
    if not math.isfinite(m):
        raise ValueError("heads_panel: non-finite weight")
    sw = 13 - math.frexp(m)[1] + 1 if m > 0.0 else 0
    sw = max(-100, min(100, sw))
    panel = torch.empty(int(_lib.lib().ocn_heads_panel_bytes(N, K)), dtype=torch.uint8, device=w.device)
    check(_lib.lib().ocn_heads_split_weight(ptr(w), N, K, float(2.0 ** sw), ptr(panel), stream_ptr()), "ocn_heads_split_weight")
    return panel, float(2.0 ** -sw)


HEADS_WIDTHS = (128, 256)
train_linear = True
train_tails = os.environ.get("OCN_TRAIN_TAILS", "1") != "0"
fused_heads = True
fused_heads_min_width = 128


def heads_small_batch(max_rows: int = -1) -> int:
    return int(_lib.lib().ocn_heads_small_batch(int(max_rows)))


@_on_device
def heads_fused(x1: Tensor, x2: Tensor, xij: Tensor, pack: dict, ranges: Optional[Tensor], y_row_map: Optional[Tensor],
                b_on_union: bool, scratch: Tensor, dump: Optional[Tensor] = None) -> Optional[Tensor]:
    for t, nm in ((x1, "xcn1"), (x2, "xcn2"), (xij, "xij")):
        _req(t, torch.float32, nm, 2)
    B, H = xij.shape
    if x1.shape != (B, H) or x2.shape != (B, H) or H not in HEADS_WIDTHS:
        raise ValueError("heads_fused: shape mismatch")
    a = _lib.OcnHeadsArgs()
    a.x[0], a.x[1], a.x[2] = x1.data_ptr(), x2.data_ptr(), xij.data_ptr()
    a.ldx, a.B, a.H = H, B, H
    for i in range(3):
        a.p_first[i] = pack["first"][i].data_ptr()
        a.p_out[i] = pack["out"][i].data_ptr()
    a.p_mid[0], a.p_mid[1] = pack["mid"][0].data_ptr(), pack["mid"][1].data_ptr()
    a.vec = pack["vec"].data_ptr()
    a.ranges = 0 if ranges is None else _req(ranges, torch.int64, "ranges").data_ptr()
    a.y_row_map = 0 if y_row_map is None else _req(y_row_map, torch.int64, "y_row_map", 1).data_ptr()
    y = None
    nconst = int(_lib.lib().ocn_heads_const_bytes(H)) // 4
    if dump is None:
        y = torch.empty((B, 1), dtype=torch.float32, device=xij.device)
        a.y = y.data_ptr()
        if _req(pack["cpark"], torch.float32, "cpark", 1).numel() != nconst:
            raise ValueError("heads_fused: constants buffer of the wrong size")
        a.cpark = pack["cpark"].data_ptr()
    else:
        if B != 1 or _req(dump, torch.float32, "dump", 1).numel() != nconst:
            raise ValueError("heads_fused: constants mode takes one row and ocn_heads_const_bytes(H) bytes")
        a.dump = dump.data_ptr()
    if scratch.numel() * scratch.element_size() < int(_lib.lib().ocn_heads_scratch_bytes(H)):
        raise ValueError("heads_fused: scratch too small")
    a.scratch = scratch.data_ptr()
    a.eps, a.ln, a.b_on_union = float(pack["eps"]), int(pack["ln"]), int(bool(b_on_union))
    _mark("mlp_glue")
    check(_lib.lib().ocn_heads_fused(ctypes.byref(a), stream_ptr()), "ocn_heads_fused")
    _mark("linear", pack["flops_per_row"] * B)
    return y


def linear_ok(x: Tensor, weight: Tensor) -> bool:
    return (fast_linear and x.is_cuda and x.dim() == 2 and x.dtype == torch.float32 and x.is_contiguous()
            and weight.shape[0] in LINEAR_WIDTHS and weight.shape[1] % 16 == 0 and weight.shape[1] == x.shape[1])


@_on_device
def linear(x: Tensor, weight: Tensor, bias: Optional[Tensor] = None, ln=None, relu: bool = False,
           dot=None, y_row_map: Optional[Tensor] = None) -> Tensor:
    _req(x, torch.float32, "x", 2)
    M, K = x.shape
    N = weight.shape[0]
    if y_row_map is not None:
        if dot is None:
            raise ValueError("y_row_map needs the dot epilogue")
        y = torch.empty((M, 1), dtype=torch.float32, device=x.device)
        linear_grouped([dict(x=x, weight=weight, bias=bias, ln=ln, relu=relu, dot=(dot[0].reshape(1, -1), dot[1]), y=y,
                             y_row_map=y_row_map)], K, N)
        return y
    panel = linear_panel(weight)
    _mark("mlp_glue")
    y = torch.empty((M, 1) if dot is not None else (M, N), dtype=torch.float32, device=x.device)
    g = b = None
    eps = 0.0
    if ln is not None:
        g, b, eps = ln
    dw = db = None
    if dot is not None:
        dw, db = dot
        dw = dw.reshape(-1)
    check(_lib.lib().ocn_linear_bf16x6(ptr(x), M, K, ptr(panel), N, ptr(bias), ptr(g), ptr(b), float(eps),
                                       int(relu), ptr(dw), ptr(db), ptr(y), stream_ptr()), "ocn_linear_bf16x6")
    _mark("linear", 2.0 * M * K * N)
    return y


def linear_ok_t(gy: Tensor, weight: Tensor) -> bool:
    return (fast_linear and gy.is_cuda and gy.dim() == 2 and gy.dtype == torch.float32
            and weight.shape[1] in LINEAR_WIDTHS and weight.shape[0] % 16 == 0 and weight.shape[0] == gy.shape[1])


@_on_device
def linear_t(gy: Tensor, weight: Tensor) -> Tensor:
    gy = _req(gy.contiguous(), torch.float32, "gy", 2)
    wt = _req(weight.detach().t().contiguous(), torch.float32, "weight^T", 2)
    K, N = wt.shape
    M = gy.shape[0]
    panel = torch.empty(int(_lib.lib().ocn_linear_panel_bytes(K, N)), dtype=torch.uint8, device=wt.device)
    check(_lib.lib().ocn_linear_split_weight(ptr(wt), K, N, ptr(panel), stream_ptr()), "ocn_linear_split_weight")
    y = torch.empty((M, K), dtype=torch.float32, device=gy.device)
# ... 106 lines not shown
```

### ocn_amd/utils.py

```python
from __future__ import annotations

from typing import Optional, Tuple

import torch
from torch import Tensor

from . import ops
from .sparse import SparseTensor


class PermIterator:

    def __init__(self, device, size, bs, training=True) -> None:
        self.bs = bs
        self.training = training
        self.idx = torch.randperm(size, device=device) if training else torch.arange(size, device=device)

    def __len__(self):
        return (self.idx.shape[0] + (self.bs - 1) * (not self.training)) // self.bs

    def __iter__(self):
        self.ptr = 0
        return self

    def __next__(self):
        if self.ptr + self.bs * self.training > self.idx.shape[0]:
            raise StopIteration
        ret = self.idx[self.ptr:self.ptr + self.bs]
        self.ptr += self.bs
        return ret


class CNState:

    def __init__(self, adj: SparseTensor, t1: Optional[SparseTensor], t2: Optional[SparseTensor],
                 tarei: Tensor, walk: bool = False, ws: Optional[dict] = None):
        if tarei.dim() != 2 or tarei.shape[0] != 2:
            raise ValueError("tarei must be [2, B]")
        for t in (t1, t2):
            if t is not None and t.sparse_sizes() != adj.sparse_sizes():
                raise ValueError("adjoverlap: adjacency sizes differ")
        if walk and adj.size(0) != adj.size(1):
            raise ValueError("get_cn1_cn2 needs a square adjacency")
        self.adj, self.walk, self.t2 = adj, walk, t2
        self.ws = ws
        self.src = tarei[0].to(torch.int64).contiguous()
        self.dst = tarei[1].to(torch.int64).contiguous()
        self.B = self.src.numel()
        self.N = adj.size(1)
        ops.check_edges(self.src, self.dst, adj.size(0), adj.size(0) if walk else t1.size(0))
        self.rec = None if (walk or self.B == 0) else ops.buf(ws, "rec", (self.B, 4), torch.int64, self.src.device)
        self.sched = (ops.buf(ws, "sched", 2 * ((self.B + 3) // 4), torch.int32, self.src.device)
                      if (self.rec is not None and ops.heavy_first and self.B >= ops.sort_edges_min_batch) else None)
        t2_rows = (t2 is not None and not walk and t2.rows_on_demand() and not getattr(ops, "_overlap_active", False))
        (self.order, self.off, self.flags, self.wc, self.hist, self.cnt1, self.cnt2, self.status, self.scal) = ops.cn_flags(
            adj._rowptr, adj._col, None if walk else (t1._rowptr, t1._col),
            None if (walk or t2 is None) else ((None, None) if t2_rows else
                                               (t2._rowptr, t2._col if (t2.col_materialized() or t2._bitmap is None) else None)),
            self.src, self.dst, self.N,
            adj.max_rowcount(), walk=walk,
            t2_bitmap=None if (walk or t2 is None) else (t2.product_bit_rows(self.dst) if t2_rows else t2.product_bit_rows()), wsd=ws,
            nds=adj.neighbor_degree_sum() if (walk and ops.walk_two_sided) else None,
            t1_bitmap=None if walk else t1.bit_rows(), rec=self.rec, sched=self.sched)
        self._hist_live = True

    @classmethod
    def from_materialized(cls, adj: SparseTensor, cn1: SparseTensor, cn2: SparseTensor, tarei: Tensor,
                          ws: Optional[dict] = None) -> "CNState":
        st = cls.__new__(cls)
        st.adj, st.ws = adj, ws
        st.src = tarei[0].to(torch.int64).contiguous()
        st.dst = tarei[1].to(torch.int64).contiguous()
        st.B, st.N = st.src.numel(), adj.size(1)
        dev = st.src.device
        if tuple(cn1.sizes()) != (st.B, st.N) or tuple(cn2.sizes()) != (st.B, st.N):
            raise ValueError("cn1 / cn2 must be [B, N] with B = tar_ei.shape[1], N = adj.size(1)")
        ops.check_edges(st.src, st.dst, adj.size(0), adj.size(0))
        st.order = None
        st.off = ops.edge_offsets(adj._rowptr, st.src)
        total = int(st.off[-1])
        st.flags = torch.zeros(max(total, 1), dtype=torch.uint8, device=dev)
        rows_sel = adj[st.src]
        r_s, c_s, _ = rows_sel.coo()
        key_s = r_s * st.N + c_s
        v2 = cn2.storage.value()
        st.walk = bool(v2 is not None and v2.numel() and bool((v2 != 1).any()))
        st.wc = torch.zeros(max(total, 1), dtype=torch.int32, device=dev) if st.walk else None
        for bit, m in ((1, cn1), (2, cn2)):
            r, c, v = m.coo()
            key = r * st.N + c
            pos = torch.searchsorted(key_s, key).clamp_(max=max(key_s.numel() - 1, 0))
            if key.numel() and not bool((key_s[pos] == key).all()):
                raise NotImplementedError("cn1 / cn2 entries outside the source rows of `adj` cannot be expressed as CN flags")
            if bit == 2 and v is not None:
                keep = v != 0
                pos, v = pos[keep], v[keep]
            st.flags[pos] |= bit
            if bit == 2 and st.walk:
                st.wc[pos] = v.to(torch.int32)
        f = st.flags[:total].to(torch.int64)
        e_of = r_s
        st.cnt1 = torch.zeros(st.B, dtype=torch.int64, device=dev).index_add_(0, e_of, f & 1).to(torch.int32)
        st.cnt2 = torch.zeros(st.B, dtype=torch.int64, device=dev).index_add_(0, e_of, (f >> 1) & 1).to(torch.int32)
        z = torch.zeros(st.N, dtype=torch.int64, device=dev)
        n1 = z.clone().index_add_(0, c_s, f & 1)
        n2 = z.clone().index_add_(0, c_s, (f >> 1) & 1)
        nu = z.clone().index_add_(0, c_s, (f != 0).to(torch.int64))
        walks = z.clone().index_add_(0, c_s, st.wc[:total].to(torch.int64)) if st.walk else z
        st.hist = torch.stack([n1 | (n2 << ops.HIST_FIELD_BITS) | (nu << (2 * ops.HIST_FIELD_BITS)), walks], dim=1).contiguous()
        st.status = torch.zeros(4, dtype=torch.int32, device=dev)
        st.scal = torch.zeros(4, dtype=torch.int32, device=dev)
        st._hist_live = True
        return st

    def check_status(self) -> None:
        bits = int(self.status[0].item())
        if bits:
            self.status[3:].zero_()
            raise RuntimeError(ops.status_message(bits))

    def hist_counts(self) -> Tensor:
        assert self._hist_live, "histogram already consumed"
        return ops.hist_counts(self.hist)

    def weights_cn5(self, innerprod: Tensor) -> Tensor:
        assert self._hist_live, "histogram already consumed"
        self._hist_live = False
        s2, scal = None, self.scal
        if ops.colsum_wanted(innerprod):
            run = lambda init: ops.cn_colsum_exact(self.adj._rowptr, self.adj._col, self.src, self.off, self.flags, None,
                                                   self.wc, self.hist, innerprod, scal, self.ws, s2_init=init)[0]
            if getattr(self, "sharded", False):
                from .dist import ring_colsum
                s2 = ring_colsum(run, self.hist.shape[0], self.hist.device, self.shard_group)
            else:
                s2 = run(None)
        return ops.cn_weights_cn5(self.hist, innerprod, valued=self.walk, wsd=self.ws, s2_exact=s2, scal=scal)

    def weights_cn7(self, sum_fill: float, diag1: Optional[Tensor] = None, diag2: Optional[Tensor] = None) -> Tensor:
        assert self._hist_live, "histogram already consumed"
        self._hist_live = False
        return ops.cn_weights_cn7(self.hist, sum_fill, diag1, diag2)

    def gather(self, weights: Tensor, h: Tensor, order: Optional[Tensor] = None, out_row: Optional[Tensor] = None,
               rowsum: Optional[Tensor] = None):
        return ops.cn_gather(self.adj._rowptr, self.adj._col, self.src, self.dst, self.off,
                             self.flags, self.wc, weights, h, order=self.order if order is None else order,
                             max_row_len=self.adj.max_rowcount(), wsd=self.ws, out_row=out_row,
                             cnt1=self.cnt1, cnt2=self.cnt2, rec=getattr(self, "rec", None) if order is None else None,
                             sched=getattr(self, "sched", None) if order is None else None,
                             rowsum=None if self.walk else rowsum, sched_ready=getattr(self, "_sched_ready", False))

    def prepare_schedule(self, H: int) -> None:
        if H == 256 and getattr(self, "sched", None) is not None and getattr(self, "rec", None) is not None:
            self._sched_ready = ops.gather_schedule(self.sched, self.B)

    def gather_backward(self, weights: Tensor, h: Tensor, g1: Tensor, g2: Tensor, g3: Tensor) -> Tensor:
        return ops.cn_gather_backward(self.adj._rowptr, self.adj._col, self.src, self.dst, self.off, self.flags,
                                      self.wc, weights, h, g1.contiguous(), g2.contiguous(), g3.contiguous(),
                                      order=self.order)

    def cn5_batch_innerprod(self) -> Tensor:
        hc = self.hist_counts()
        if self.walk:
            n1 = hc[:, 0]
            inv1 = torch.where(n1 >= 2, 1.0 / n1.clamp(min=1).to(torch.float32), torch.zeros((), device=n1.device))
            both = self.materialize(1)
            r, c, _ = both.coo()
            cn2 = self.materialize(2)
            key2 = cn2.coo()[0] * self.N + cn2.coo()[1]
            key1 = r * self.N + c
            idx = torch.searchsorted(key2, key1).clamp(max=max(key2.numel() - 1, 0))
            hit = (key2[idx] == key1) if key2.numel() else torch.zeros_like(key1, dtype=torch.bool)
            return (cn2.storage.value()[idx[hit]] * inv1[c[hit]]).sum()
        n1 = hc[:, 0]
        nb = n1 + hc[:, 1] - hc[:, 2]
        inv1 = torch.where(n1 >= 2, 1.0 / n1.clamp(min=1).to(torch.float32), torch.zeros((), device=n1.device))
        return (nb.to(torch.float32) * inv1).sum()

    def materialize(self, bit: int) -> SparseTensor:
        row_sel = self.adj[self.src]
        r, c, _ = row_sel.coo()
        pos = torch.arange(r.numel(), device=r.device) - row_sel._rowptr[:-1][r] + self.off[:-1][r]
        keep = (self.flags[pos] & bit) != 0
        val = torch.ones(int(keep.sum()), device=r.device)
        if self.walk and bit == 2:
            val = self.wc[pos][keep].to(torch.float32)
        return SparseTensor(row=r[keep], col=c[keep], value=val, sparse_sizes=(self.B, self.N),
                            is_sorted=True, trust_data=True)


class CNBatch:

    def __init__(self, adj1: SparseTensor, adj2: Optional[SparseTensor], tarei: Tensor, mode: str = "pattern"):
        self.adj1, self.adj2, self.tarei, self.mode = adj1, adj2, tarei, mode
        self._state: Optional[CNState] = None

    def sizes(self):
        return [self.tarei.shape[1], self.adj1.size(1)]

    def size(self, dim: int) -> int:
        return self.sizes()[dim]

    def device(self):
# ... 11 lines not shown
        st = self._single()
        return st.cnt2 if self.mode == "walk2" else st.cnt1

    def materialize(self) -> SparseTensor:
        return self._single().materialize(2 if self.mode == "walk2" else 1)


class CNState3:

    def __init__(self, adj: SparseTensor, adj2: SparseTensor, adj3: SparseTensor, tarei: Tensor):
        self.a = CNState(adj, adj, adj2, tarei)
        self.b = CNState(adj, adj3, None, tarei)
        self.adj, self.B, self.N = adj, self.a.B, self.a.N

    @property
    def cnt3(self) -> Tensor:
        return self.b.cnt1

    def weights(self, innerprod: Tensor, sharded: bool = False):
        assert self.a._hist_live and self.b._hist_live, "histograms already consumed"
        self.a._hist_live = self.b._hist_live = False
        exact = None if sharded else (self.adj._rowptr, self.adj._col, self.a.src, self.a.off, self.a.flags, self.b.flags)
        return ops.cn_weights_cn6(self.a.hist, self.b.hist, innerprod, exact=exact, scal=self.a.scal)

    def gather(self, wa: Tensor, wb: Tensor, nip: Tensor, h: Tensor):
        return ops.cn_gather3(self.adj._rowptr, self.adj._col, self.a.src, self.a.dst, self.a.off, self.a.flags,
                              self.b.flags, wa, wb, nip, h, order=self.a.order)

    def gather_backward(self, wa: Tensor, wb: Tensor, nip: Tensor, h: Tensor, g1, g2, g3, g4) -> Tensor:
        return ops.cn_gather3_backward(self.adj._rowptr, self.adj._col, self.a.src, self.a.dst, self.a.off, self.a.flags,
                                       self.b.flags, wa, wb, nip, h, g1.contiguous(), g2.contiguous(), g3.contiguous(),
                                       g4.contiguous(), order=self.a.order)


def _same_edges(a: Tensor, b: Tensor) -> bool:
    if a is b or (a.data_ptr() == b.data_ptr() and a.shape == b.shape and a.stride() == b.stride()
                  and a.dtype == b.dtype and a.device == b.device):
        return True
    return torch.equal(a, b)


def fuse3(cn1: "CNBatch", cn2: "CNBatch", cn3: "CNBatch", tar_ei: Tensor) -> CNState3:
    for c in (cn1, cn2, cn3):
        if not isinstance(c, CNBatch) or c.mode != "pattern":
            raise NotImplementedError("cn6 takes the handles returned by ocn_amd.utils.adjoverlap")
    if not (cn1.adj1 is cn2.adj1 is cn3.adj1) or cn1.adj2 is not cn1.adj1:
        raise NotImplementedError("cn1/cn2/cn3 must come from adjoverlap(adj, adj|adj2|adj3, e) of one adjacency")
    if ops.validate_indices and not (_same_edges(cn1.tarei, cn2.tarei) and _same_edges(cn1.tarei, cn3.tarei)
                                     and _same_edges(cn1.tarei, tar_ei)):
        raise NotImplementedError("cn1, cn2, cn3 and tar_ei must be built from the same candidate edges")
    return CNState3(cn1.adj1, cn2.adj2, cn3.adj2, cn1.tarei)


def fuse(cn1, cn2, tar_ei: Tensor, ws: Optional[dict] = None, adj: Optional[SparseTensor] = None) -> CNState:
    if isinstance(cn1, CNBatch) != isinstance(cn2, CNBatch):
        cn1 = cn1.materialize() if isinstance(cn1, CNBatch) else cn1
        cn2 = cn2.materialize() if isinstance(cn2, CNBatch) else cn2
    if isinstance(cn1, SparseTensor) and isinstance(cn2, SparseTensor):
        if not isinstance(adj, SparseTensor):
            raise TypeError("explicit cn1 / cn2 matrices need the adjacency (the predictor's `adj` argument) to be rebuilt "
                            "as CN flags")
        return CNState.from_materialized(adj, cn1, cn2, tar_ei, ws=None)
    if not isinstance(cn1, CNBatch) or not isinstance(cn2, CNBatch):
        raise TypeError("ocn_amd predictors take the CNBatch handles returned by ocn_amd.utils.adjoverlap "
                        "/ get_cn1_cn2, or explicit [B, N] SparseTensors")
    if cn1.adj1 is not cn2.adj1:
        raise NotImplementedError("cn1 and cn2 must select their source rows from the same adjacency")
    if cn1.tarei.shape != cn2.tarei.shape or cn1.tarei.shape != tar_ei.shape:
        raise ValueError("cn1, cn2 and tar_ei describe different numbers of candidate edges")
    if ops.validate_indices and not (_same_edges(cn1.tarei, cn2.tarei) and _same_edges(cn1.tarei, tar_ei)):
        raise NotImplementedError("cn1, cn2 and tar_ei must be built from the same candidate edges")
    if cn1.mode == "walk1" and cn2.mode == "walk2":
        return CNState(cn1.adj1, None, None, cn1.tarei, walk=True, ws=ws)
    if cn1.mode != "pattern" or cn2.mode != "pattern":
        raise NotImplementedError("mixing adjoverlap and get_cn1_cn2 handles in one predictor call")
    return CNState(cn1.adj1, cn1.adj2, cn2.adj2, cn1.tarei, ws=ws)


class CN8State:

    def __init__(self, adj: SparseTensor, t1: SparseTensor, t2: SparseTensor, tarei: Tensor, ws: Optional[dict] = None):
        if tarei.dim() != 2 or tarei.shape[0] != 2:
            raise ValueError("tarei must be [2, B]")
        for t in (t1, t2):
            if t.sparse_sizes() != adj.sparse_sizes():
                raise ValueError("adjoverlap: adjacency sizes differ")
        self.adj, self.t1, self.t2, self.ws = adj, t1, t2, ws
        self.src = tarei[0].to(torch.int64).contiguous()
        self.dst = tarei[1].to(torch.int64).contiguous()
        self.B, self.N = self.src.numel(), adj.size(1)
        self.walk = False
        self.cnt1 = self.cnt2 = self.order = None

    def pool(self, h: Tensor):
        adj, t1, t2 = self.adj, self.t1, self.t2
        if h.dim() != 2 or h.shape[0] != self.N:
            raise ValueError("h must have one row per column of the adjacency")
        lazy = t2.rows_on_demand() and not getattr(ops, "_overlap_active", False)
        bm2 = t2.product_bit_rows(self.dst) if lazy else t2.product_bit_rows()
        csr2 = None if bm2 is not None else (t2._rowptr, t2._col)
        bm1 = t1.bit_rows()
        if self.B >= ops.sort_edges_min_batch:
            self.order = ops.order_by_node(self.src, adj.size(0), self.ws)
        x1, x2, xij, self.cnt1, self.cnt2 = ops.cn8_pool(adj._rowptr, adj._col, (t1._rowptr, t1._col), csr2, self.src, self.dst, h,
                                                         t1_bitmap=bm1, t2_bitmap=bm2, order=self.order, wsd=self.ws, n_cols=self.N)
        return x1, x2, xij


def fuse8(cn1, cn2, tar_ei: Tensor, ws: Optional[dict] = None) -> Optional[CN8State]:
    if not (isinstance(cn1, CNBatch) and isinstance(cn2, CNBatch) and cn1.mode == "pattern" and cn2.mode == "pattern"):
        return None
    if cn1.adj1 is not cn2.adj1:
        raise NotImplementedError("cn1 and cn2 must select their source rows from the same adjacency")
    if cn1.tarei.shape != cn2.tarei.shape or cn1.tarei.shape != tar_ei.shape:
        raise ValueError("cn1, cn2 and tar_ei describe different numbers of candidate edges")
    if ops.validate_indices and not (_same_edges(cn1.tarei, cn2.tarei) and _same_edges(cn1.tarei, tar_ei)):
        raise NotImplementedError("cn1, cn2 and tar_ei must be built from the same candidate edges")
    return CN8State(cn1.adj1, cn1.adj2, cn2.adj2, cn1.tarei, ws=ws)


def adjoverlap(adj1: SparseTensor, adj2: SparseTensor, tarei: Tensor, filled1: bool = False,
               calresadj: bool = False, cnsampledeg: int = -1, ressampledeg: int = -1) -> CNBatch:
    if calresadj or cnsampledeg > 0 or ressampledeg > 0:
        raise NotImplementedError("calresadj / neighbour sampling are outside the cn5/cn7 path")
    return CNBatch(adj1, adj2, tarei)


def get_cn1_cn2(adj: SparseTensor, tedge: Tensor) -> Tuple[CNBatch, CNBatch]:
    return CNBatch(adj, None, tedge, "walk1"), CNBatch(adj, None, tedge, "walk2")
# ... 22 lines not shown
```

Measured before the change: 171.6 million.

## Compute xij product inside CN flags kernel and map rows in fused heads

Adds an option to compute the elementwise h[i]*h[j] product inside the intersection-flags kernel, written in batch order, so the gather kernel can skip that work and skip edges that have no common neighbours. The fused heads kernel gains an x_row_map so it can read xij in batch order while the other branches use the sorted order. The flags kernel is also pinned to 8 waves per EU. The new path is gated behind OCN_XIJ_IN_FLAGS, which defaults off, though the waves-per-EU attribute applies to every launch.

Result: slower. 168.1 million (-2.0%).

```diff
diff --git a/include/ocn_hip.h b/include/ocn_hip.h
--- a/include/ocn_hip.h
+++ b/include/ocn_hip.h
@@ -71,6 +71,16 @@
                      int64_t n_cols, const int64_t* off, uint8_t* flags, int64_t flags_cap,
                      uint64_t* hist , int32_t* cnt1, int32_t* cnt2,
                      int32_t* status, uint64_t* rec , int32_t* gcost , void* stream);
+int ocn_cn_flags_xij(const int64_t* rowptrA, const int32_t* colA,
+                     const int64_t* rowptrT1, const int32_t* colT1,
+                     const int64_t* rowptrT2, const int32_t* colT2,
+                     const uint32_t* bitmapT1 , int64_t bm1_stride_words,
+                     const uint32_t* bitmapT2 , int64_t bm_stride_words,
+                     const int64_t* src, const int64_t* dst, const int64_t* order, int64_t B,
+                     int64_t n_cols, const int64_t* off, uint8_t* flags, int64_t flags_cap,
+                     uint64_t* hist , int32_t* cnt1, int32_t* cnt2,
+                     int32_t* status, uint64_t* rec, int32_t* gcost , int32_t rec_in,
+                     const float* h, int32_t H, float* xij , void* stream);
 
 int32_t ocn_walk_chunk(void);
 int ocn_cn_walk_flags(const int64_t* rowptrA, const int32_t* colA, const int64_t* nds ,
@@ -290,6 +300,7 @@
 int64_t ocn_heads_panel_bytes(int32_t N, int32_t K);
 int ocn_heads_split_weight(const float* W, int32_t N, int32_t K, float scale, void* Wp, void* stream);
 int ocn_heads_fused(const OcnHeadsArgs* args, void* stream);
+int ocn_heads_fused_xmap(const OcnHeadsArgs* args, const int64_t* x_row_map , void* stream);
 int64_t ocn_heads_small_batch(int64_t max_rows);
 
 int64_t ocn_coo_to_csr_workspace_bytes(int64_t nnz, int64_t n_rows, int32_t symmetrize, int32_t dedupe);
diff --git a/ocn_amd/_lib.py b/ocn_amd/_lib.py
--- a/ocn_amd/_lib.py
+++ b/ocn_amd/_lib.py
@@ -31,6 +31,8 @@
                                _P, _P, _P, _P, _P, _P]),
     "ocn_cn_flags_rec": (c_int32, [_P, _P, _P, _P, _P, _P, _P, c_int64, _P, c_int64, _P, _P, _P, c_int64, c_int64, _P, _P, c_int64, _P,
                                    _P, _P, _P, _P, _P, _P]),
+    "ocn_cn_flags_xij": (c_int32, [_P, _P, _P, _P, _P, _P, _P, c_int64, _P, c_int64, _P, _P, _P, c_int64, c_int64, _P, _P, c_int64, _P,
+                                   _P, _P, _P, _P, _P, c_int32, _P, c_int32, _P, _P]),
     "ocn_chunk_offsets": (c_int32, [_P, _P, _P, _P, c_int64, _P, _P, _P]),
     "ocn_walk_chunk": (c_int32, []),
     "ocn_cn_walk_flags": (c_int32, [_P, _P, _P, _P, _P, _P, c_int64, _P, _P, _P, c_int64, _P, _P, c_int64, _P, _P, _P,
@@ -113,6 +115,7 @@
     "ocn_heads_panel_bytes": (c_int64, [c_int32, c_int32]),
     "ocn_heads_split_weight": (c_int32, [_P, c_int32, c_int32, c_float, _P, _P]),
     "ocn_heads_fused": (c_int32, [_P, _P]),
+    "ocn_heads_fused_xmap": (c_int32, [_P, _P, _P]),
     "ocn_heads_small_batch": (c_int64, [c_int64]),
 }
 
diff --git a/ocn_amd/csrc/cn_stage.hip b/ocn_amd/csrc/cn_stage.hip
--- a/ocn_amd/csrc/cn_stage.hip
+++ b/ocn_amd/csrc/cn_stage.hip
@@ -53,7 +53,7 @@
 }
 
 template <bool HAS_T2, bool LH, bool RECIN>
-__global__ __launch_bounds__(OCN_BLOCK) void cn_flags_kernel(
+__global__ __launch_bounds__(OCN_BLOCK) __attribute__((amdgpu_waves_per_eu(8, 8))) void cn_flags_kernel(
     const i64* __restrict__ rowptrA, const int32_t* __restrict__ colA,
     const i64* __restrict__ rowptrT1, const int32_t* __restrict__ colT1,
     const i64* __restrict__ rowptrT2, const int32_t* __restrict__ colT2,
@@ -61,7 +61,8 @@
     const i64* __restrict__ src, const i64* __restrict__ dst, const i64* __restrict__ order, i64 B,
     i64 n_cols, const i64* __restrict__ off, uint8_t* __restrict__ flags, i64 cap,
     u64* __restrict__ hist, int32_t* __restrict__ cnt1, int32_t* __restrict__ cnt2,
-    int32_t* __restrict__ status, u64* rec, int32_t* __restrict__ gcost) {
+    int32_t* __restrict__ status, u64* rec, int32_t* __restrict__ gcost,
+    const float* __restrict__ h, int H, float* __restrict__ xij) {
   constexpr int GPB = OCN_WPB;
   __shared__ int s_cost[2][GPB];
   __shared__ int32_t s_t1[GPB][T1_CAP];
@@ -109,10 +110,27 @@
     else if (t1_lds)
       for (i64 q = gl; q < db; q += OCN_WAVE) s_t1[g][q] = colT1[b0 + q];
     const bool t2_full = HAS_T2 && rowptrT2 && dc == n_cols;
+    int32_t t2v = 0;
+    bool t2w = false;
     if (HAS_T2 && !t2_full && !bmT2) {
-      if (dc > OCN_WAVE) s_t2[g][gl] = colT2[c0 + (((i64)gl * dc) >> 6)];
-      else if (gl < dc) s_t2[g][gl] = colT2[c0 + gl];
-    }
+      t2w = dc > OCN_WAVE || gl < dc;
+      if (dc > OCN_WAVE) t2v = colT2[c0 + (((i64)gl * dc) >> 6)];
+      else if (gl < dc) t2v = colT2[c0 + gl];
+    }
+    const i64 rowq = H >> 2;
+    const bool xl = xij && act && gl < rowq;
+    float4 xa, xb;
+    unsigned xo = (unsigned)gl * 16u;
+    asm volatile("" : "+v"(xo));
+    if (xl) {
+      const char* hb = reinterpret_cast<const char*>(h);
+      xa = *reinterpret_cast<const float4*>(hb + wave_uniform(i) * rowq * 16 + xo);
+      xb = *reinterpret_cast<const float4*>(hb + wave_uniform(j) * rowq * 16 + xo);
+    }
+    if (t2w) s_t2[g][gl] = t2v;
+    if (xl)
+      *reinterpret_cast<float4*>(reinterpret_cast<char*>(xij) + wave_uniform(e) * rowq * 16 + xo) =
+          make_float4(__fmul_rn(xa.x, xb.x), __fmul_rn(xa.y, xb.y), __fmul_rn(xa.z, xb.z), __fmul_rn(xa.w, xb.w));
     wave_lds_sync();
     const bool fits = base + da <= cap;
     int c1 = 0, c2 = 0;
@@ -644,10 +662,18 @@
                                            const float4 (&acc1)[NV], const float4 (&acc2)[NV],
                                            float* __restrict__ xcn1, float* __restrict__ xcn2,
                                            float* __restrict__ xij, bool st1 = true, bool st2 = true) {
+  float4* o1 = reinterpret_cast<float4*>(xcn1) + e * rowq + gl;
+  float4* o2 = reinterpret_cast<float4*>(xcn2) + e * rowq + gl;
+  if (!xij) {
+#pragma unroll
+    for (int v = 0; v < NV; ++v) {
+      if (st1) o1[v * LPE] = acc1[v];
+      if (st2) o2[v * LPE] = acc2[v];
+    }
+    return;
+  }
   const float4* hi = h4 + i * rowq + gl;
   const float4* hj = h4 + j * rowq + gl;
-  float4* o1 = reinterpret_cast<float4*>(xcn1) + e * rowq + gl;
-  float4* o2 = reinterpret_cast<float4*>(xcn2) + e * rowq + gl;
   float4* o3 = reinterpret_cast<float4*>(xij) + e * rowq + gl;
 #pragma unroll
   for (int v = 0; v < NV; ++v) {
@@ -667,7 +693,8 @@
     const i64* __restrict__ src, const i64* __restrict__ dst, const i64* __restrict__ order, i64 B,
     const i64* __restrict__ off, const uint8_t* __restrict__ flags, const int32_t* __restrict__ wc,
     const float4* __restrict__ weights, const float* __restrict__ h, int H,
-    float* __restrict__ xcn1, float* __restrict__ xcn2, float* __restrict__ xij,
+    float* __restrict__ xcn1, float* __restrict__ xcn2,
+    float* __restrict__ xij,
     const i64* __restrict__ out_row,
     const int32_t* __restrict__ cnt1, const int32_t* __restrict__ cnt2,
     const u64* __restrict__ rec,
@@ -702,6 +729,7 @@
     full2 = rowsum && cnt2 && da > 0 && (i64)cnt2[e] == da;
   }
   if (da > LONG_ROW && !full2) return;
+  if (!xij && out_row && !has1 && !has2) return;
   const float4* h4 = reinterpret_cast<const float4*>(h);
   const i64 rowq = H >> 2;
   float4 acc1[NV], acc2[NV];
@@ -987,7 +1015,7 @@
     for (int q = 0; q < FPL; ++q) {
       xcn1[o + q] = acc1[q];
       xcn2[o + q] = acc2[q];
-      xij[o + q] = __fmul_rn(h[i * H + lane * FPL + q], h[j * H + lane * FPL + q]);
+      if (xij) xij[o + q] = __fmul_rn(h[i * H + lane * FPL + q], h[j * H + lane * FPL + q]);
     }
   }
 }
@@ -1318,8 +1346,10 @@
                            const uint32_t* bitmapT1, int64_t bm1_stride_words, const uint32_t* bitmapT2, int64_t bm_stride_words,
                            const int64_t* src, const int64_t* dst, const int64_t* order, int64_t B,
                            int64_t n_cols, const int64_t* off, uint8_t* flags, int64_t flags_cap, uint64_t* hist,
-                           int32_t* cnt1, int32_t* cnt2, int32_t* status, uint64_t* rec, int32_t* gcost, bool rec_in, void* stream) {
+                           int32_t* cnt1, int32_t* cnt2, int32_t* status, uint64_t* rec, int32_t* gcost, bool rec_in,
+                           const float* h, int32_t H, float* xij, void* stream) {
   if (B < 0 || flags_cap < 0 || B > (int64_t)HF_MASK) return OCN_EINVAL;
+  if (xij && (!h || H <= 0 || (H & 3) || H > 4 * OCN_WAVE)) return OCN_EINVAL;
   if (B == 0) return 0;
   if (!rowptrA || (!rowptrT1 && !bitmapT1) || !src || !dst || !off || !hist || !cnt1 || !status) return OCN_EINVAL;
   if (rec_in && (!rec || !order)) return OCN_EINVAL;
@@ -1348,7 +1378,7 @@
   (const i64*)rowptrA, colA, (const i64*)rowptrT1, colT1, (const i64*)(T2P), (T2C),                   \
       (const unsigned*)bitmapT1, (i64)bm1_stride_words, (const unsigned*)bitmapT2, (i64)bm_stride_words, (const i64*)src, \
       (const i64*)dst, (const i64*)order, (i64)B, (i64)n_cols, (const i64*)off, flags, (i64)flags_cap, \
-      (u64*)hist, cnt1, cnt2, status, (u64*)rec, gcost
+      (u64*)hist, cnt1, cnt2, status, (u64*)rec, gcost, h, (int)H, xij
 #define CN_FLAGS_LAUNCH(T2, LHV, RI, T2P, T2C)                                                        \
   hipLaunchKernelGGL((cn_flags_kernel<T2, LHV, RI>), dim3(grid), dim3(OCN_BLOCK), (LHV) ? lds : 0, st, CN_FLAGS_ARGS(T2P, T2C))
 #define CN_FLAGS_PICK(T2, T2P, T2C)                                                                   \
@@ -1371,7 +1401,8 @@
                  int64_t n_cols, const int64_t* off, uint8_t* flags, int64_t flags_cap, uint64_t* hist,
                  int32_t* cnt1, int32_t* cnt2, int32_t* status, uint64_t* rec, int32_t* gcost, void* stream) {
   return cn_flags_launch(rowptrA, colA, rowptrT1, colT1, rowptrT2, colT2, bitmapT1, bm1_stride_words, bitmapT2, bm_stride_words,
-                         src, dst, order, B, n_cols, off, flags, flags_cap, hist, cnt1, cnt2, status, rec, gcost, false, stream);
+                         src, dst, order, B, n_cols, off, flags, flags_cap, hist, cnt1, cnt2, status, rec, gcost, false,
+                         nullptr, 0, nullptr, stream);
 }
 
 int ocn_cn_flags_rec(const int64_t* rowptrA, const int32_t* colA, const int64_t* rowptrT1,
@@ -1381,7 +1412,21 @@
                      int64_t n_cols, const int64_t* off, uint8_t* flags, int64_t flags_cap, uint64_t* hist,
                      int32_t* cnt1, int32_t* cnt2, int32_t* status, uint64_t* rec, int32_t* gcost, void* stream) {
   return cn_flags_launch(rowptrA, colA, rowptrT1, colT1, rowptrT2, colT2, bitmapT1, bm1_stride_words, bitmapT2, bm_stride_words,
-                         src, dst, order, B, n_cols, off, flags, flags_cap, hist, cnt1, cnt2, status, rec, gcost, true, stream);
+                         src, dst, order, B, n_cols, off, flags, flags_cap, hist, cnt1, cnt2, status, rec, gcost, true,
+                         nullptr, 0, nullptr, stream);
+}
+
+int ocn_cn_flags_xij(const int64_t* rowptrA, const int32_t* colA, const int64_t* rowptrT1,
+                     const int32_t* colT1, const int64_t* rowptrT2, const int32_t* colT2,
+                     const uint32_t* bitmapT1, int64_t bm1_stride_words, const uint32_t* bitmapT2, int64_t bm_stride_words,
+                     const int64_t* src, const int64_t* dst, const int64_t* order, int64_t B,
+                     int64_t n_cols, const int64_t* off, uint8_t* flags, int64_t flags_cap, uint64_t* hist,
+                     int32_t* cnt1, int32_t* cnt2, int32_t* status, uint64_t* rec, int32_t* gcost, int32_t rec_in,
+                     const float* h, int32_t H, float* xij, void* stream) {
+  if (!h || !xij) return OCN_EINVAL;
+  return cn_flags_launch(rowptrA, colA, rowptrT1, colT1, rowptrT2, colT2, bitmapT1, bm1_stride_words, bitmapT2, bm_stride_words,
+                         src, dst, order, B, n_cols, off, flags, flags_cap, hist, cnt1, cnt2, status, rec, gcost, rec_in != 0,
+                         h, H, xij, stream);
 }
 
 int ocn_cn_walk_flags(const int64_t* rowptrA, const int32_t* colA, const int64_t* nds, const int64_t* src,
@@ -1521,7 +1566,8 @@
                   void* stream) {
   if (B < 0 || H <= 0) return OCN_EINVAL;
   if (B == 0) return 0;
-  if (!rowptrA || !src || !dst || !off || !weights || !h || !xcn1 || !xcn2 || !xij) return OCN_EINVAL;
+  if (!rowptrA || !src || !dst || !off || !weights || !h || !xcn1 || !xcn2) return OCN_EINVAL;
+  if (!xij && H != 128 && H != 256 && H != 512) return OCN_EINVAL;
   if (rowsum && (wc || !cnt2)) return OCN_EINVAL;
   hipStream_t st = (hipStream_t)stream;
   switch (H) {
diff --git a/ocn_amd/csrc/heads.hip b/ocn_amd/csrc/heads.hip
--- a/ocn_amd/csrc/heads.hip
+++ b/ocn_amd/csrc/heads.hip
@@ -20,6 +20,7 @@
   const float* vec;
   const i64* ranges;
   const i64* y_row_map;
+  const i64* x_row_map;
   float* y;
   float* dump;
   const float* cpark;
@@ -342,8 +343,14 @@
     return true;
   };
   auto x_row = [&](i64 tl, int br) -> const float* {
-    const i64 slot = tl * HD_ROWS + 32 * w + r;
-    return a.x[br] + (slot < a.B ? slot : a.B - 1) * a.ldx + 4 * hh;
+    i64 row = tl * HD_ROWS + 32 * w + r;
+    row = row < a.B ? row : a.B - 1;
+    const bool mapped = br == 2 && a.x_row_map;
+    const i64* mp = mapped ? a.x_row_map + row : reinterpret_cast<const i64*>(a.vec);
+    i64 mrow;
+    asm volatile("global_load_dwordx2 %0, %1, off\n\ts_waitcnt vmcnt(0)" : "=&v"(mrow) : "v"(mp) : "memory");
+    row = mapped ? mrow : row;
+    return a.x[br] + row * a.ldx + 4 * hh;
   };
   auto first_branch = [&](i64 tl) -> int { return tile_runs(tl, 0) ? 0 : (tile_runs(tl, 1) ? 1 : 2); };
 
@@ -719,7 +726,9 @@
 #pragma unroll
     for (int br = 0; br < 3; ++br) {
       if (!(br == 0 ? wgA : (br == 1 ? wgB : true))) continue;
-      const float* xr = a.x[br] + (live ? slot : a.B - 1) * a.ldx + 4 * hh + 32 * (w * TW);
+      i64 row = live ? slot : a.B - 1;
+      if (br == 2 && a.x_row_map) row = a.x_row_map[row];
+      const float* xr = a.x[br] + row * a.ldx + 4 * hh + 32 * (w * TW);
 #pragma unroll
       for (int u = 0; u < TW; ++u)
 #pragma unroll
@@ -916,7 +925,7 @@
 
 int64_t ocn_heads_scratch_bytes(int32_t H) { return HD_PARK_BYTES(H) + 4096; }
 
-int ocn_heads_fused(const OcnHeadsArgs* h, void* stream) {
+static int heads_fused_launch(const OcnHeadsArgs* h, const int64_t* x_row_map, void* stream) {
   if (!h || h->B < 0 || h->H <= 0) return OCN_EINVAL;
   if (h->B == 0) return 0;
   for (int i = 0; i < 3; ++i)
@@ -931,6 +940,7 @@
   a.panel[P_B0] = (const char*)h->p_first[1]; a.panel[P_B3] = (const char*)h->p_mid[1]; a.panel[P_MB] = (const char*)h->p_out[1];
   a.panel[P_X0] = (const char*)h->p_first[2]; a.panel[P_MC] = (const char*)h->p_out[2];
   a.ldx = ldx; a.B = h->B; a.vec = h->vec; a.ranges = (const i64*)h->ranges; a.y_row_map = (const i64*)h->y_row_map;
+  a.x_row_map = (const i64*)x_row_map;
   a.y = h->y; a.dump = h->dump; a.cpark = h->cpark; a.scratch = h->scratch; a.eps = h->eps; a.ln = h->ln; a.b_on_union = h->b_on_union;
   const i64 tiles = h->dump ? 1 : (h->B + HD_ROWS - 1) / HD_ROWS;
   hipStream_t st = (hipStream_t)stream;
@@ -946,4 +956,10 @@
   }
 }
 
-}
+int ocn_heads_fused(const OcnHeadsArgs* h, void* stream) { return heads_fused_launch(h, nullptr, stream); }
+
+int ocn_heads_fused_xmap(const OcnHeadsArgs* h, const int64_t* x_row_map, void* stream) {
+  return heads_fused_launch(h, x_row_map, stream);
+}
+
+}
diff --git a/ocn_amd/model.py b/ocn_amd/model.py
--- a/ocn_amd/model.py
+++ b/ocn_amd/model.py
@@ -582,7 +582,7 @@
         n_sets = max(2, int(ops.overlap_depth), int(ops.overlap_depth_small))
         if len(getattr(self, "_ws_slots", ())) != n_sets:
             self._ws_slots = [dict() for _ in range(n_sets)]
-        st = fuse(cn1, cn2, tar_ei, self._ws_slots[slot % n_sets], adj=adj)
+        st = fuse(cn1, cn2, tar_ei, self._ws_slots[slot % n_sets], adj=adj, xij_h=self._xij_early(x))
         handle = None
         if self._sharded:
             from .dist import allreduce_hist_start
@@ -619,7 +619,14 @@
             w = w_early if w_early is not None else self._weights(st, args)
             pooled = self._pool(st, w, x)
         xcn1, xcn2, xij = pooled
-        return self._heads(x, xcn1, xcn2, xij, getattr(st, "cls", None))
+        return self._heads(x, xcn1, xcn2, xij, getattr(st, "cls", None), getattr(st, "xij", None) is not None)
+
+    def _xij_early(self, x):
+        if (ops.xij_in_flags and not self.training and not torch.is_grad_enabled() and torch.is_tensor(x) and x.is_cuda
+                and x.dim() == 2 and x.dtype == torch.float32 and x.is_contiguous() and x.shape[0] > 0
+                and x.shape[1] >= ops.fused_heads_min_width and self._fused_plan(x.shape[1]) is not None):
+            return x
+        return None
 
     def check_errors(self) -> None:
         words = [t for d in ([self._ws] + list(getattr(self, "_ws_slots", ()))) for k, t in d.items() if k[0] == "status"]
@@ -904,19 +911,22 @@
         self._fpack, self._fpack_key = pack, key
         return pack
 
-    def _heads_fused(self, xcn1, xcn2, xij, cls):
+    def _heads_fused(self, xcn1, xcn2, xij, cls, xij_batch_order=False):
         B, H = xij.shape
         pack = self._fused_pack(H, xij.device)
         scratch = ops.buf(self._ws, "heads_scratch", int(ops._lib.lib().ocn_heads_scratch_bytes(H)) // 4, torch.float32, xij.device)
         ranges, rowmap = (None, None) if cls is None else (cls[2], cls[0])
-        return ops.heads_fused(xcn1, xcn2, xij, pack, ranges, rowmap, self._xcn2_on_union, scratch)
-
-    def _heads(self, x, xcn1, xcn2, xij, cls=None):
+        return ops.heads_fused(xcn1, xcn2, xij, pack, ranges, rowmap, self._xcn2_on_union, scratch,
+                               xij_batch_order=xij_batch_order)
+
+    def _heads(self, x, xcn1, xcn2, xij, cls=None, xij_batch_order=False):
         if (not self.training and not torch.is_grad_enabled() and xij.is_cuda and xij.dim() == 2 and xij.shape[0] > 0
                 and xij.is_contiguous() and xcn1.is_contiguous() and xcn2.is_contiguous()
                 and xcn1.shape == xij.shape and xij.shape[1] >= ops.fused_heads_min_width
                 and self._fused_plan(xij.shape[1]) is not None):
-            return self._heads_fused(xcn1, xcn2, xij, cls)
+            return self._heads_fused(xcn1, xcn2, xij, cls, xij_batch_order)
+        if xij_batch_order and cls is not None:
+            raise RuntimeError("x_i * x_j in batch order beside class-major pooled rows: only the fused head reads that")
         if cls is not None:
             return self._heads_skipping(xcn1, xcn2, xij, cls)
         if self.training or torch.is_grad_enabled() or not xij.is_cuda or xij.shape[-1] % 4:
@@ -940,10 +950,10 @@
 
     def multidomainforward(self, x, adj, cn1, cn2, tar_ei, filled1: bool = False,
                            cndropprobs: Iterable[float] = []):
-        st = self._exchange(fuse(cn1, cn2, tar_ei, self._scratch(x), adj=adj), x)
+        st = self._exchange(fuse(cn1, cn2, tar_ei, self._scratch(x), adj=adj, xij_h=self._xij_early(x)), x)
         w = self._weights(st, None)
         xcn1, xcn2, xij = self._pool(st, w, x)
-        return self._heads(x, xcn1, xcn2, xij, getattr(st, "cls", None))
+        return self._heads(x, xcn1, xcn2, xij, getattr(st, "cls", None), getattr(st, "xij", None) is not None)
 
     def _weights(self, st, args):
         return st.weights_cn5(self.innerprod1(st))
@@ -960,10 +970,10 @@
 
     def multidomainforward(self, x, adj, cn1, cn2, tar_ei, args, filled1: bool = False,
                            cndropprobs: Iterable[float] = []):
-        st = self._exchange(fuse(cn1, cn2, tar_ei, self._scratch(x), adj=adj), x)
+        st = self._exchange(fuse(cn1, cn2, tar_ei, self._scratch(x), adj=adj, xij_h=self._xij_early(x)), x)
         w = self._weights(st, args)
         xcn1, xcn2, xij = self._pool(st, w, x)
-        return self._heads(x, xcn1, xcn2, xij, getattr(st, "cls", None))
+        return self._heads(x, xcn1, xcn2, xij, getattr(st, "cls", None), getattr(st, "xij", None) is not None)
 
     def _weights(self, st, args):
         dev = st.hist.device
diff --git a/ocn_amd/ops.py b/ocn_amd/ops.py
--- a/ocn_amd/ops.py
+++ b/ocn_amd/ops.py
@@ -200,7 +200,8 @@
 def cn_flags(rowptrA: Tensor, colA: Tensor, t1: Optional[Tuple[Tensor, Tensor]],
              t2: Optional[Tuple[Tensor, Tensor]], src: Tensor, dst: Tensor, n_cols: int, max_deg_a: int,
              walk: bool = False, t2_bitmap: Optional[Tensor] = None, wsd=None, nds: Optional[Tensor] = None,
-             t1_bitmap: Optional[Tensor] = None, rec: Optional[Tensor] = None, sched: Optional[Tensor] = None):
+             t1_bitmap: Optional[Tensor] = None, rec: Optional[Tensor] = None, sched: Optional[Tensor] = None,
+             xij: Optional[Tuple[Tensor, Tensor]] = None):
     dev = src.device
     B = src.numel()
     _req(rowptrA, torch.int64, "rowptrA", 1); _req(colA, torch.int32, "colA", 1)
@@ -216,6 +217,10 @@
         raise ValueError("src/dst length mismatch")
     if B > MAX_BATCH:
         raise ValueError(f"candidate batch of {B} edges exceeds the histogram field width ({MAX_BATCH})")
+    if xij is not None:
+        xh, xo = _req(xij[0], torch.float32, "h", 2), _req(xij[1], torch.float32, "xij", 2)
+        if walk or xo.shape != (B, xh.shape[1]) or xh.shape[1] % 4 or xh.shape[1] > 256 or xh.shape[0] < rowptrA.numel() - 1:
+            raise ValueError("xij: (h [N, H], out [B, H]) with H <= 256, pattern route only")
     _mark("begin")
     if walk and 0 < B <= int(_lib.lib().ocn_walk_prep_max_batch()) and walk_share_min > 0:
         return _cn_flags_walk_small(rowptrA, colA, src, dst, n_cols, max_deg_a, wsd, nds)
@@ -284,12 +289,17 @@
             _req(t1_bitmap, torch.int32, "t1_bitmap", 2)
             if t1_bitmap.shape[0] != t1[0].numel() - 1 or t1_bitmap.shape[1] * 32 < n_cols:
                 raise ValueError("t1_bitmap does not match the T1 adjacency")
-        check((_lib.lib().ocn_cn_flags_rec if rec_in else _lib.lib().ocn_cn_flags)(ptr(rowptrA), ptr(colA), ptr(t1[0]), ptr(t1[1]),
-                                      ptr(t2[0] if t2 else None), ptr(t2[1] if t2 else None),
-                                      ptr(t1_bitmap), t1_bitmap.shape[1] if t1_bitmap is not None else 0,
-                                      ptr(t2_bitmap), t2_bitmap.shape[1] if t2_bitmap is not None else 0,
-                                      ptr(src), ptr(dst), ptr(order), B, n_cols, ptr(off), ptr(flags), cap, ptr(hist),
-                                      ptr(cnt1), ptr(cnt2), ptr(status), ptr(rec), ptr(sched), stream_ptr()), "ocn_cn_flags")
+        args = (ptr(rowptrA), ptr(colA), ptr(t1[0]), ptr(t1[1]),
+                ptr(t2[0] if t2 else None), ptr(t2[1] if t2 else None),
+                ptr(t1_bitmap), t1_bitmap.shape[1] if t1_bitmap is not None else 0,
+                ptr(t2_bitmap), t2_bitmap.shape[1] if t2_bitmap is not None else 0,
+                ptr(src), ptr(dst), ptr(order), B, n_cols, ptr(off), ptr(flags), cap, ptr(hist),
+                ptr(cnt1), ptr(cnt2), ptr(status), ptr(rec), ptr(sched))
+        if xij is not None and B > 0:
+            check(_lib.lib().ocn_cn_flags_xij(*args, int(rec_in), ptr(xij[0]), xij[0].shape[1], ptr(xij[1]), stream_ptr()),
+                  "ocn_cn_flags_xij")
+        else:
+            check((_lib.lib().ocn_cn_flags_rec if rec_in else _lib.lib().ocn_cn_flags)(*args, stream_ptr()), "ocn_cn_flags")
     _mark("cn_flags")
     return order, off, flags, wc, hist, cnt1, cnt2, status, scal
 
@@ -418,13 +428,16 @@
 def cn_gather(rowptrA, colA, src, dst, off, flags, wc: Optional[Tensor], weights: Tensor, h: Tensor,
               order: Optional[Tensor] = None, max_row_len: int = 0, wsd=None, out_row: Optional[Tensor] = None,
               cnt1: Optional[Tensor] = None, cnt2: Optional[Tensor] = None, rec: Optional[Tensor] = None,
-              sched: Optional[Tensor] = None, rowsum: Optional[Tensor] = None, sched_ready: bool = False):
+              sched: Optional[Tensor] = None, rowsum: Optional[Tensor] = None, sched_ready: bool = False,
+              xij: Optional[Tensor] = None):
     _req(weights, torch.float32, "weights", 2)
     _req(h, torch.float32, "h", 2)
     if weights.shape[0] != h.shape[0] or weights.shape[1] != 4:
         raise ValueError("weights must be [N,4] with N = h.shape[0]")
     B, H = src.numel(), h.shape[1]
     out = buf(wsd, "pooled", (3, B, H), torch.float32, h.device)
+    if xij is not None and (_req(xij, torch.float32, "xij", 2).shape != (B, H) or H not in (128, 256, 512)):
+        raise ValueError("xij: [B, H] rows of the intersection pass, H in {128, 256, 512}")
     if rowsum is not None and (wc is not None or cnt2 is None or _req(rowsum, torch.float32, "rowsum", 2).shape != h.shape):
         raise ValueError("rowsum: [N, H] row sums of h, pattern route with per-row counts only")
     perm = None
@@ -436,10 +449,10 @@
     _mark("cn_pre")
     check(_lib.lib().ocn_cn_gather(ptr(rowptrA), ptr(colA), ptr(src), ptr(dst), ptr(order), B, ptr(off), ptr(flags),
                                    ptr(wc), ptr(weights), ptr(h), H, int(max_row_len), ptr(out[0]), ptr(out[1]),
-                                   ptr(out[2]), ptr(out_row), ptr(cnt1), ptr(cnt2), ptr(rec), ptr(perm), ptr(rowsum),
-                                   stream_ptr()), "ocn_cn_gather")
+                                   ptr(out[2] if xij is None else None), ptr(out_row), ptr(cnt1), ptr(cnt2), ptr(rec), ptr(perm),
+                                   ptr(rowsum), stream_ptr()), "ocn_cn_gather")
     _mark("cn_gather")
-    return out[0], out[1], out[2]
+    return out[0], out[1], out[2] if xij is None else xij
 
 
 _unit_w: dict = {}
@@ -1185,6 +1198,7 @@
 train_linear = True
 train_tails = os.environ.get("OCN_TRAIN_TAILS", "1") != "0"
 fused_heads = True
+xij_in_flags = os.environ.get("OCN_XIJ_IN_FLAGS", "0") == "1"
 fused_heads_min_width = 128
 
 
@@ -1194,7 +1208,7 @@
 
 @_on_device
 def heads_fused(x1: Tensor, x2: Tensor, xij: Tensor, pack: dict, ranges: Optional[Tensor], y_row_map: Optional[Tensor],
-                b_on_union: bool, scratch: Tensor, dump: Optional[Tensor] = None) -> Optional[Tensor]:
+                b_on_union: bool, scratch: Tensor, dump: Optional[Tensor] = None, xij_batch_order: bool = False) -> Optional[Tensor]:
     for t, nm in ((x1, "xcn1"), (x2, "xcn2"), (xij, "xij")):
         _req(t, torch.float32, nm, 2)
     B, H = xij.shape
@@ -1227,7 +1241,10 @@
     a.scratch = scratch.data_ptr()
     a.eps, a.ln, a.b_on_union = float(pack["eps"]), int(pack["ln"]), int(bool(b_on_union))
     _mark("mlp_glue")
-    check(_lib.lib().ocn_heads_fused(ctypes.byref(a), stream_ptr()), "ocn_heads_fused")
+    if xij_batch_order and y_row_map is not None:
+        check(_lib.lib().ocn_heads_fused_xmap(ctypes.byref(a), ptr(y_row_map), stream_ptr()), "ocn_heads_fused_xmap")
+    else:
+        check(_lib.lib().ocn_heads_fused(ctypes.byref(a), stream_ptr()), "ocn_heads_fused")
     _mark("linear", pack["flops_per_row"] * B)
     return y
 
diff --git a/ocn_amd/utils.py b/ocn_amd/utils.py
--- a/ocn_amd/utils.py
+++ b/ocn_amd/utils.py
@@ -34,7 +34,7 @@
 class CNState:
 
     def __init__(self, adj: SparseTensor, t1: Optional[SparseTensor], t2: Optional[SparseTensor],
-                 tarei: Tensor, walk: bool = False, ws: Optional[dict] = None):
+                 tarei: Tensor, walk: bool = False, ws: Optional[dict] = None, xij_h: Optional[Tensor] = None):
         if tarei.dim() != 2 or tarei.shape[0] != 2:
             raise ValueError("tarei must be [2, B]")
         for t in (t1, t2):
@@ -52,6 +52,10 @@
         self.rec = None if (walk or self.B == 0) else ops.buf(ws, "rec", (self.B, 4), torch.int64, self.src.device)
         self.sched = (ops.buf(ws, "sched", 2 * ((self.B + 3) // 4), torch.int32, self.src.device)
                       if (self.rec is not None and ops.heavy_first and self.B >= ops.sort_edges_min_batch) else None)
+        self.xij, self.xij_h = None, None
+        if xij_h is not None and not walk and self.B > 0:
+            self.xij_h = xij_h
+            self.xij = ops.buf(ws, "pooled", (3, self.B, xij_h.shape[1]), torch.float32, self.src.device)[2]
         t2_rows = (t2 is not None and not walk and t2.rows_on_demand() and not getattr(ops, "_overlap_active", False))
         (self.order, self.off, self.flags, self.wc, self.hist, self.cnt1, self.cnt2, self.status, self.scal) = ops.cn_flags(
             adj._rowptr, adj._col, None if walk else (t1._rowptr, t1._col),
@@ -61,7 +65,8 @@
             adj.max_rowcount(), walk=walk,
             t2_bitmap=None if (walk or t2 is None) else (t2.product_bit_rows(self.dst) if t2_rows else t2.product_bit_rows()), wsd=ws,
             nds=adj.neighbor_degree_sum() if (walk and ops.walk_two_sided) else None,
-            t1_bitmap=None if walk else t1.bit_rows(), rec=self.rec, sched=self.sched)
+            t1_bitmap=None if walk else t1.bit_rows(), rec=self.rec, sched=self.sched,
+            xij=None if self.xij is None else (self.xij_h, self.xij))
         self._hist_live = True
 
     @classmethod
@@ -144,12 +149,15 @@
 
     def gather(self, weights: Tensor, h: Tensor, order: Optional[Tensor] = None, out_row: Optional[Tensor] = None,
                rowsum: Optional[Tensor] = None):
+        xij = getattr(self, "xij", None)
+        if xij is not None and h is not self.xij_h:
+            raise ValueError("the pooling was handed other embeddings than the intersection pass multiplied")
         return ops.cn_gather(self.adj._rowptr, self.adj._col, self.src, self.dst, self.off,
                              self.flags, self.wc, weights, h, order=self.order if order is None else order,
                              max_row_len=self.adj.max_rowcount(), wsd=self.ws, out_row=out_row,
                              cnt1=self.cnt1, cnt2=self.cnt2, rec=getattr(self, "rec", None) if order is None else None,
                              sched=getattr(self, "sched", None) if order is None else None,
-                             rowsum=None if self.walk else rowsum, sched_ready=getattr(self, "_sched_ready", False))
+                             rowsum=None if self.walk else rowsum, sched_ready=getattr(self, "_sched_ready", False), xij=xij)
 
     def prepare_schedule(self, H: int) -> None:
         if H == 256 and getattr(self, "sched", None) is not None and getattr(self, "rec", None) is not None:
@@ -267,7 +275,8 @@
     return CNState3(cn1.adj1, cn2.adj2, cn3.adj2, cn1.tarei)
 
 
-def fuse(cn1, cn2, tar_ei: Tensor, ws: Optional[dict] = None, adj: Optional[SparseTensor] = None) -> CNState:
+def fuse(cn1, cn2, tar_ei: Tensor, ws: Optional[dict] = None, adj: Optional[SparseTensor] = None,
+         xij_h: Optional[Tensor] = None) -> CNState:
     if isinstance(cn1, CNBatch) != isinstance(cn2, CNBatch):
         cn1 = cn1.materialize() if isinstance(cn1, CNBatch) else cn1
         cn2 = cn2.materialize() if isinstance(cn2, CNBatch) else cn2
@@ -289,7 +298,7 @@
         return CNState(cn1.adj1, None, None, cn1.tarei, walk=True, ws=ws)
     if cn1.mode != "pattern" or cn2.mode != "pattern":
         raise NotImplementedError("mixing adjoverlap and get_cn1_cn2 handles in one predictor call")
-    return CNState(cn1.adj1, cn1.adj2, cn2.adj2, cn1.tarei, ws=ws)
+    return CNState(cn1.adj1, cn1.adj2, cn2.adj2, cn1.tarei, ws=ws, xij_h=xij_h)
 
 
 class CN8State:
```
